# bioinformatics-ua/polus

Hardware: AMD Instinct MI355X
Metric: train samples/sec BioBERT-base NER seq256 (higher is better)
Workload: dtype bf16

## Files before the change

### polus_amd/csrc/attention.hip

```cpp
#include "common.h"

namespace {

constexpr int D = 64;
constexpr int BLK = 64;
constexpr float MASK_NEG = -10000.0f;
constexpr float LOG2E = 1.4426950408889634f, LN2 = 0.6931471805599453f;

template <typename T> struct TileCfg;
template <> struct TileCfg<bf16_t> { static constexpr int RS = 160, EPC = 8, LOG_CPR = 3, NLOAD = 2; };
template <> struct TileCfg<float> { static constexpr int RS = 288, EPC = 4, LOG_CPR = 4, NLOAD = 4; };

template <typename T, int NT = 256>
__device__ __forceinline__ void tile_load(unsigned char* tile, const T* __restrict__ base, long ld, int row0,
                                          int nrows, int col0, int tid) {
    constexpr int LOG = TileCfg<T>::LOG_CPR;
#pragma unroll
    for (int k = 0; k < TileCfg<T>::NLOAD; ++k) {
        int c = tid + NT * k;
        int r = c >> LOG, ch = c & ((1 << LOG) - 1);
        uint4 v = make_uint4(0, 0, 0, 0);
        if (row0 + r < nrows)
            v = *reinterpret_cast<const uint4*>(base + (long)(row0 + r) * ld + col0 + ch * TileCfg<T>::EPC);
        *reinterpret_cast<uint4*>(tile + r * TileCfg<T>::RS + ch * 16) = v;
    }
}

template <typename T>
__device__ __forceinline__ void frag_global(Frag<T>& f, const T* __restrict__ p, bool valid);
template <>
__device__ __forceinline__ void frag_global<bf16_t>(Frag<bf16_t>& f, const bf16_t* __restrict__ p, bool valid) {
    uint4 v = make_uint4(0, 0, 0, 0);
    if (valid) v = *reinterpret_cast<const uint4*>(p);
    f.v = __builtin_bit_cast(bf16x8, v);
}
template <>
__device__ __forceinline__ void frag_global<float>(Frag<float>& f, const float* __restrict__ p, bool valid) {
    float4 a = make_float4(0, 0, 0, 0), b = a;
    if (valid) { a = *reinterpret_cast<const float4*>(p); b = *reinterpret_cast<const float4*>(p + 4); }
    f.v[0] = a.x; f.v[1] = a.y; f.v[2] = a.z; f.v[3] = a.w;
    f.v[4] = b.x; f.v[5] = b.y; f.v[6] = b.z; f.v[7] = b.w;
}

template <typename T>
__device__ __forceinline__ void frag_row(Frag<T>& f, const unsigned char* tile, int row, int sub, int g) {
    frag_load_row(f, tile + row * TileCfg<T>::RS + (sub * 32 + 8 * g) * (int)sizeof(T));
}

__device__ __forceinline__ void frag_tr(Frag<bf16_t>& f, const unsigned char* tile, int kb, int d0, int i, int g) {
    const unsigned char* p = tile + (kb + 4 * g + (i >> 2)) * 160 + (d0 + 4 * (i & 3)) * 2;
    s16x4 lo = lds_tr16(p);
    s16x4 hi = lds_tr16(p + 16 * 160);
    typedef short s16x8 __attribute__((ext_vector_type(8)));
    s16x8 w = {lo[0], lo[1], lo[2], lo[3], hi[0], hi[1], hi[2], hi[3]};
    f.v = __builtin_bit_cast(bf16x8, w);
}
__device__ __forceinline__ void frag_tr(Frag<float>& f, const unsigned char* tile, int kb, int d0, int i, int g) {
#pragma unroll
    for (int j = 0; j < 8; ++j)
        f.v[j] = *reinterpret_cast<const float*>(tile + (kb + 16 * (j >> 2) + 4 * g + (j & 3)) * 288 + (d0 + i) * 4);
}

__device__ __forceinline__ void frag_from_acc(Frag<bf16_t>& f, const f32x4& t0, const f32x4& t1) {
    f.v[0] = (bf16_t)t0[0]; f.v[1] = (bf16_t)t0[1]; f.v[2] = (bf16_t)t0[2]; f.v[3] = (bf16_t)t0[3];
    f.v[4] = (bf16_t)t1[0]; f.v[5] = (bf16_t)t1[1]; f.v[6] = (bf16_t)t1[2]; f.v[7] = (bf16_t)t1[3];
}
__device__ __forceinline__ void frag_from_acc(Frag<float>& f, const f32x4& t0, const f32x4& t1) {
    f.v[0] = t0[0]; f.v[1] = t0[1]; f.v[2] = t0[2]; f.v[3] = t0[3];
    f.v[4] = t1[0]; f.v[5] = t1[1]; f.v[6] = t1[2]; f.v[7] = t1[3];
}

__device__ __forceinline__ float col_max(float v) { v = fmaxf(v, __shfl_xor(v, 16, 64)); return fmaxf(v, __shfl_xor(v, 32, 64)); }
__device__ __forceinline__ float col_sum(float v) { v += __shfl_xor(v, 16, 64); return v + __shfl_xor(v, 32, 64); }

template <typename T>
__device__ __forceinline__ void store_acc_T(T* __restrict__ out, long ld, int row, int col0, const f32x4 (&o)[4],
                                            float mul, int g, bool valid) {
    if (!valid) return;
#pragma unroll
    for (int dt = 0; dt < 4; ++dt) {
        float v[4] = {o[dt][0] * mul, o[dt][1] * mul, o[dt][2] * mul, o[dt][3] * mul};
        store4<T>(out + (long)row * ld + col0 + dt * 16 + 4 * g, v);
    }
}

struct AttnArgs {
    const void* qkv; const int32_t* mask; void* ctx; float* lse;
    const void* dctx; const float* delta; void* dqkv;
    int B, S, A, H;
    float scale;
    unsigned drop_thresh, drop_seed;
    float drop_inv;
    const PolusDyn* dyn;
    int debug;
};

__device__ __forceinline__ float key_bias(const int32_t* mask, int b, int S, int key) {
    if (key >= S) return -INFINITY;
    if (!mask) return 0.0f;
    return (1.0f - (float)mask[(long)b * S + key]) * MASK_NEG;
}

template <typename T, int NW>
__global__ __launch_bounds__(64 * NW) void attn_fwd_kernel(AttnArgs p) {
    if (p.drop_thresh) p.drop_seed = polus_eff_seed(p.drop_seed, p.dyn);
    constexpr int QB = 16 * NW, NT = 64 * NW;
    extern __shared__ __attribute__((aligned(16))) unsigned char smem[];
    unsigned char* Kc = smem;
    unsigned char* Vc = smem + QB * TileCfg<T>::RS;
    float* kbc = reinterpret_cast<float*>(smem + 2 * QB * TileCfg<T>::RS);
    const int tid = threadIdx.x, lane = tid & 63, wid = tid >> 6, i = lane & 15, g = lane >> 4;
    const int q0 = blockIdx.x * QB, h = blockIdx.y, b = blockIdx.z;
    const int S = p.S, H = p.H;
    const long ld = 3L * H;
    const T* qkv = static_cast<const T*>(p.qkv) + (long)b * S * ld;
    const int q = q0 + wid * 16 + i;
    const bool qvalid = q < S;

    Frag<T> qf[2];
#pragma unroll
    for (int sub = 0; sub < 2; ++sub)
        frag_global<T>(qf[sub], qkv + (long)q * ld + h * D + sub * 32 + 8 * g, qvalid);

    const float scale2 = p.scale * LOG2E;
    float m = -1e30f, l = 0.f;
    f32x4 o[4];
#pragma unroll
    for (int dt = 0; dt < 4; ++dt) o[dt] = (f32x4){0.f, 0.f, 0.f, 0.f};

    for (int kc0 = 0; kc0 < S; kc0 += QB) {
        __syncthreads();
        tile_load<T, NT>(Kc, qkv, ld, kc0, S, H + h * D, tid);
        tile_load<T, NT>(Vc, qkv, ld, kc0, S, 2 * H + h * D, tid);
        if (tid < QB) kbc[tid] = key_bias(p.mask, b, S, kc0 + tid) * LOG2E;
        __syncthreads();
      for (int kb0 = kc0; kb0 < kc0 + QB && kb0 < S; kb0 += BLK) {
        const unsigned char* Kt = Kc + (kb0 - kc0) * TileCfg<T>::RS;
        const unsigned char* Vt = Vc + (kb0 - kc0) * TileCfg<T>::RS;
        const float* kbias = kbc + (kb0 - kc0);

        f32x4 s[4];
#pragma unroll
        for (int kt = 0; kt < 4; ++kt) {
            s[kt] = (f32x4){0.f, 0.f, 0.f, 0.f};
#pragma unroll
            for (int sub = 0; sub < 2; ++sub) {
                Frag<T> a;
                frag_row<T>(a, Kt, kt * 16 + i, sub, g);
                mma16(s[kt], a, qf[sub]);
            }
        }
        float mx = -INFINITY;
#pragma unroll
        for (int kt = 0; kt < 4; ++kt)
#pragma unroll
            for (int r = 0; r < 4; ++r) {
                s[kt][r] = fmaf(s[kt][r], scale2, kbias[kt * 16 + 4 * g + r]);
                mx = fmaxf(mx, s[kt][r]);
            }
        mx = col_max(mx);
        const float m_new = fmaxf(m, mx);
        const float alpha = __builtin_amdgcn_exp2f(m - m_new);
        float rs = 0.f;
#pragma unroll
        for (int kt = 0; kt < 4; ++kt)
#pragma unroll
            for (int r = 0; r < 4; ++r) { s[kt][r] = __builtin_amdgcn_exp2f(s[kt][r] - m_new); rs += s[kt][r]; }
        rs = col_sum(rs);
        l = l * alpha + rs;
        m = m_new;
#pragma unroll
        for (int dt = 0; dt < 4; ++dt)
#pragma unroll
            for (int r = 0; r < 4; ++r) o[dt][r] *= alpha;
        if (p.drop_thresh) {
            const unsigned rowb = (((unsigned)b * p.A + h) * S + (unsigned)q) * S + kb0 + 4 * g;
#pragma unroll
            for (int kt = 0; kt < 4; ++kt) {
                float t4[4] = {s[kt][0], s[kt][1], s[kt][2], s[kt][3]};
                polus_dropout_run<4>(t4, p.drop_seed, rowb + kt * 16, p.drop_thresh, p.drop_inv, (S & 3) == 0);
                s[kt] = (f32x4){t4[0], t4[1], t4[2], t4[3]};
            }
        }
#pragma unroll
        for (int ks = 0; ks < 2; ++ks) {
            Frag<T> pb;
            frag_from_acc(pb, s[2 * ks], s[2 * ks + 1]);
#pragma unroll
            for (int dt = 0; dt < 4; ++dt) {
                Frag<T> va;
                frag_tr(va, Vt, ks * 32, dt * 16, i, g);
                mma16(o[dt], va, pb);
            }
        }
      }
    }
    T* ctx = static_cast<T*>(p.ctx) + (long)b * S * H;
    store_acc_T<T>(ctx, H, q, h * D, o, 1.0f / l, g, qvalid);
    if (qvalid && g == 0) p.lse[((long)b * p.A + h) * S + q] = m * LN2 + __logf(l);
}

typedef __attribute__((address_space(3))) void lds_void_t;
typedef const __attribute__((address_space(1))) void* gptr_t;
__device__ __forceinline__ void dma16(const void* g, unsigned char* lds) {
    __builtin_amdgcn_global_load_lds((gptr_t)g, (lds_void_t*)lds, 16, 0, 0);
}
__device__ __forceinline__ void dma4(const void* g, unsigned char* lds) {
    __builtin_amdgcn_global_load_lds((gptr_t)g, (lds_void_t*)lds, 4, 0, 0);
}
template <int N> __device__ __forceinline__ void wait_vm() { asm volatile("s_waitcnt vmcnt(%0)" :: "n"(N) : "memory"); }
__device__ __forceinline__ void wait_lgkm() { asm volatile("s_waitcnt lgkmcnt(0)" ::: "memory"); }
template <int PPW> __device__ __forceinline__ void wait_blocks_left(int left) {
    if (left >= 3) wait_vm<3 * PPW>(); else if (left == 2) wait_vm<2 * PPW>(); else if (left == 1) wait_vm<PPW>(); else wait_vm<0>();
}
__device__ __forceinline__ float xor16(float v) {
    return __builtin_bit_cast(float, __builtin_amdgcn_ds_swizzle(__builtin_bit_cast(int, v), 0x401F));
}
__device__ __forceinline__ float col_max2(float v) {
    v = fmaxf(v, xor16(v));
    return fmaxf(v, __shfl_xor(v, 32, 64));
}
__device__ __forceinline__ float col_sum2(float v) {
    v += xor16(v);
    return v + __shfl_xor(v, 32, 64);
}

constexpr int FWD_RING = 4, FWD_STAGE = 2 * BLK * 128;
constexpr int FWD_MAX_S = 1024;

template <int NW>
__global__ __launch_bounds__(64 * NW, NW == 8 ? 4 : 2) void attn_fwd_dma_kernel(AttnArgs p) {
    typedef bf16_t T;
    constexpr int QB = 16 * NW, NT = 64 * NW, PPW = 16 / NW;
    if (p.drop_thresh) p.drop_seed = polus_eff_seed(p.drop_seed, p.dyn);
    extern __shared__ __attribute__((aligned(16))) unsigned char smem[];
    unsigned char* ring = smem;
    float* kbc = reinterpret_cast<float*>(smem + FWD_RING * FWD_STAGE);
    const int tid = threadIdx.x, lane = tid & 63, i = lane & 15, g = lane >> 4;
    const int wid = __builtin_amdgcn_readfirstlane(tid >> 6);
    const int q0 = blockIdx.x * QB, h = blockIdx.y, b = blockIdx.z;
    const int S = p.S, H = p.H;
    const long ld = 3L * H;
    const T* qkv = static_cast<const T*>(p.qkv) + (long)b * S * ld;
    const int q = q0 + wid * 16 + i;
    const int r8 = lane >> 3, src_chunk = ((lane & 7) ^ r8) * 8;

    auto issue_block = [&](int j) {
        unsigned char* st = ring + (j & 3) * FWD_STAGE;
#pragma unroll
        for (int e = 0; e < PPW; ++e) {
            const int piece = wid + e * NW;
            const int row = min(j * BLK + (piece & 7) * 8 + r8, S - 1);
            dma16(qkv + (long)row * ld + (piece < 8 ? H : 2 * H) + h * D + src_chunk, st + piece * 1024);
        }
    };
    const int nblk = (S + BLK - 1) / BLK;
    if (p.mask)
        for (int k0 = wid * 64; k0 < S; k0 += 64 * NW)
            dma4(p.mask + (long)b * S + min(k0 + lane, S - 1), reinterpret_cast<unsigned char*>(kbc) + k0 * 4);
    {
        unsigned char* qs = ring + 3 * FWD_STAGE;
#pragma unroll
        for (int e = 0; e < 2; ++e) {
            const int piece = wid + e * NW;
            dma16(qkv + (long)min(q0 + piece * 8 + r8, S - 1) * ld + h * D + src_chunk, qs + piece * 1024);
        }
    }
#pragma unroll
    for (int j = 0; j < 3; ++j) if (j < nblk) issue_block(j);
    wait_blocks_left<PPW>(min(nblk, 3));
    __builtin_amdgcn_s_barrier();
    Frag<T> qf[2];
    {
        const int row = wid * 16 + i;
#pragma unroll
        for (int sub = 0; sub < 2; ++sub)
            qf[sub].v = *reinterpret_cast<const bf16x8*>(ring + 3 * FWD_STAGE + row * 128 + (((sub * 4 + g) ^ (row & 7)) * 16));
    }
    for (int t = tid; t < nblk * BLK; t += NT) {
        float bias = 0.0f;
        if (p.mask) bias = (1.0f - (float)reinterpret_cast<const int*>(kbc)[t]) * MASK_NEG;
        kbc[t] = t < S ? bias * LOG2E : -INFINITY;
    }
    wait_lgkm();
    __builtin_amdgcn_s_barrier();
    if (nblk > 3) issue_block(3);
    int issued = min(nblk, 4);

    const float scale2 = p.scale * LOG2E;
    float m = -1e30f, l = 0.f;
    f32x4 o[4];
#pragma unroll
    for (int dt = 0; dt < 4; ++dt) o[dt] = (f32x4){0.f, 0.f, 0.f, 0.f};
    const int kx = i & 7;
    const int k_off0 = i * 128 + ((g ^ kx) * 16), k_off1 = i * 128 + (((4 + g) ^ kx) * 16);
    const int vrow = 4 * g + (i >> 2), vx = vrow & 7;
    const int v_base = vrow * 128 + (i & 1) * 8, v_c = (i & 3) >> 1;

    for (int j0 = 0; j0 < nblk; j0 += 2) {
        const bool two = j0 + 1 < nblk;
        f32x4 s[2][4];
#pragma unroll
        for (int jj = 0; jj < 2; ++jj) {
            if (jj == 0 || two) {
                wait_blocks_left<PPW>(issued - 1 - (j0 + jj));
                __builtin_amdgcn_s_barrier();
                const unsigned char* Kt = ring + ((j0 + jj) & 3) * FWD_STAGE;
#pragma unroll
                for (int kt = 0; kt < 4; ++kt) {
                    s[jj][kt] = (f32x4){0.f, 0.f, 0.f, 0.f};
                    Frag<T> a0, a1;
                    a0.v = *reinterpret_cast<const bf16x8*>(Kt + kt * 2048 + k_off0);
                    a1.v = *reinterpret_cast<const bf16x8*>(Kt + kt * 2048 + k_off1);
                    mma16(s[jj][kt], a0, qf[0]);
                    mma16(s[jj][kt], a1, qf[1]);
                }
            } else {
#pragma unroll
                for (int kt = 0; kt < 4; ++kt) s[jj][kt] = (f32x4){-INFINITY, -INFINITY, -INFINITY, -INFINITY};
            }
        }
        float mx = -INFINITY;
#pragma unroll
        for (int jj = 0; jj < 2; ++jj)
            if (jj == 0 || two) {
#pragma unroll
                for (int kt = 0; kt < 4; ++kt) {
                    const f32x4 kb = *reinterpret_cast<const f32x4*>(kbc + (j0 + jj) * BLK + kt * 16 + 4 * g);
#pragma unroll
                    for (int r = 0; r < 4; ++r) s[jj][kt][r] = fmaf(s[jj][kt][r], scale2, kb[r]);
                    mx = fmaxf(mx, fmaxf(fmaxf(s[jj][kt][0], s[jj][kt][1]), fmaxf(s[jj][kt][2], s[jj][kt][3])));
                }
            }
        mx = col_max2(mx);
        const float m_new = fmaxf(m, mx);
        const float alpha = __builtin_amdgcn_exp2f(m - m_new);
        m = m_new;
        float rs = 0.f;
        Frag<T> pf[2][2];
#pragma unroll
        for (int jj = 0; jj < 2; ++jj) {
#pragma unroll
            for (int kt = 0; kt < 4; ++kt)
#pragma unroll
                for (int r = 0; r < 4; ++r) { s[jj][kt][r] = __builtin_amdgcn_exp2f(s[jj][kt][r] - m_new); rs += s[jj][kt][r]; }
            if (p.drop_thresh) {
                const unsigned rowb = (((unsigned)b * p.A + h) * S + (unsigned)q) * S + (j0 + jj) * BLK + 4 * g;
#pragma unroll
                for (int kt = 0; kt < 4; ++kt) {
                    float t4[4] = {s[jj][kt][0], s[jj][kt][1], s[jj][kt][2], s[jj][kt][3]};
                    polus_dropout_run<4>(t4, p.drop_seed, rowb + kt * 16, p.drop_thresh, p.drop_inv, (S & 3) == 0);
                    s[jj][kt] = (f32x4){t4[0], t4[1], t4[2], t4[3]};
                }
            }
            frag_from_acc(pf[jj][0], s[jj][0], s[jj][1]);
            frag_from_acc(pf[jj][1], s[jj][2], s[jj][3]);
        }
        l = l * alpha + rs;
#pragma unroll
        for (int dt = 0; dt < 4; ++dt)
#pragma unroll
            for (int r = 0; r < 4; ++r) o[dt][r] *= alpha;
#pragma unroll
        for (int jj = 0; jj < 2; ++jj) {
            if (jj == 0 || two) {
                const unsigned char* Vt = ring + ((j0 + jj) & 3) * FWD_STAGE + BLK * 128 + v_base;
#pragma unroll
                for (int ks = 0; ks < 2; ++ks)
#pragma unroll
                    for (int dt = 0; dt < 4; ++dt) {
                        const unsigned char* vp = Vt + ks * 4096 + (((2 * dt + v_c) ^ vx) * 16);
                        const s16x4 lo = lds_tr16(vp), hi = lds_tr16(vp + 16 * 128);
                        typedef short s16x8 __attribute__((ext_vector_type(8)));
                        const s16x8 w = {lo[0], lo[1], lo[2], lo[3], hi[0], hi[1], hi[2], hi[3]};
                        Frag<T> va;
                        va.v = __builtin_bit_cast(bf16x8, w);
                        mma16(o[dt], va, pf[jj][ks]);
                    }
            }
        }
        if (j0 + 4 < nblk) {
            wait_lgkm();
            __builtin_amdgcn_s_barrier();
            issue_block(j0 + 4);
            ++issued;
            if (j0 + 5 < nblk) { issue_block(j0 + 5); ++issued; }
        }
    }
    l = col_sum2(l);
    const float inv_l = 1.0f / l;
    wait_lgkm();
    __builtin_amdgcn_s_barrier();
    unsigned char* ot = ring + wid * 2048;
#pragma unroll
    for (int dt = 0; dt < 4; ++dt) {
        float v[4] = {o[dt][0] * inv_l, o[dt][1] * inv_l, o[dt][2] * inv_l, o[dt][3] * inv_l};
        store4<T>(reinterpret_cast<T*>(ot + i * 128 + (((2 * dt + (g >> 1)) ^ (i & 7)) * 16) + (g & 1) * 8), v);
    }
    wait_lgkm();
    T* ctx = static_cast<T*>(p.ctx) + (long)b * S * H;
#pragma unroll
    for (int t = 0; t < 2; ++t) {
        const int row = 8 * t + r8, qq = q0 + wid * 16 + row;
        const uint4 v = *reinterpret_cast<const uint4*>(ot + row * 128 + (lane & 7) * 16);
        if (qq < S) *reinterpret_cast<uint4*>(ctx + (long)qq * H + h * D + (((lane & 7) ^ (row & 7)) * 8)) = v;
    }
    if (q < S && g == 0) p.lse[((long)b * p.A + h) * S + q] = m * LN2 + __logf(l);
}

template <typename T, int NW>
__global__ __launch_bounds__(64 * NW) void attn_bwd_dq_kernel(AttnArgs p) {
    if (p.drop_thresh) p.drop_seed = polus_eff_seed(p.drop_seed, p.dyn);
    constexpr int QB = 16 * NW, NT = 64 * NW;
    extern __shared__ __attribute__((aligned(16))) unsigned char smem[];
    unsigned char* Kc = smem;
    unsigned char* Vc = smem + QB * TileCfg<T>::RS;
    float* kbc = reinterpret_cast<float*>(smem + 2 * QB * TileCfg<T>::RS);
    const int tid = threadIdx.x, lane = tid & 63, wid = tid >> 6, i = lane & 15, g = lane >> 4;
    const int q0 = blockIdx.x * QB, h = blockIdx.y, b = blockIdx.z;
    const int S = p.S, H = p.H;
    const long ld = 3L * H;
    const T* qkv = static_cast<const T*>(p.qkv) + (long)b * S * ld;
    const T* dctx = static_cast<const T*>(p.dctx) + (long)b * S * H;
    const int q = q0 + wid * 16 + i;
    const bool qvalid = q < S;

    Frag<T> qf[2], dof[2];
#pragma unroll
    for (int sub = 0; sub < 2; ++sub) {
        frag_global<T>(qf[sub], qkv + (long)q * ld + h * D + sub * 32 + 8 * g, qvalid);
        frag_global<T>(dof[sub], dctx + (long)q * H + h * D + sub * 32 + 8 * g, qvalid);
    }
    const long stat = ((long)b * p.A + h) * S + q;
    const float lse2 = (qvalid ? p.lse[stat] : 0.f) * LOG2E;
    const float scale2 = p.scale * LOG2E;
    float dl = 0.f;
    {
        const T* ctx = static_cast<const T*>(p.ctx) + (long)b * S * H;
#pragma unroll
        for (int sub = 0; sub < 2; ++sub) {
            Frag<T> of;
            frag_global<T>(of, ctx + (long)q * H + h * D + sub * 32 + 8 * g, qvalid);
#pragma unroll
            for (int j = 0; j < 8; ++j) dl += (float)of.v[j] * (float)dof[sub].v[j];
        }
        dl = col_sum(dl);
        if (qvalid && g == 0) const_cast<float*>(p.delta)[stat] = dl;
    }

    f32x4 dq[4];
#pragma unroll
    for (int dt = 0; dt < 4; ++dt) dq[dt] = (f32x4){0.f, 0.f, 0.f, 0.f};

    for (int kc0 = 0; kc0 < S; kc0 += QB) {
        __syncthreads();
        tile_load<T, NT>(Kc, qkv, ld, kc0, S, H + h * D, tid);
        tile_load<T, NT>(Vc, qkv, ld, kc0, S, 2 * H + h * D, tid);
        if (tid < QB) kbc[tid] = key_bias(p.mask, b, S, kc0 + tid) * LOG2E;
        __syncthreads();
      for (int kb0 = kc0; kb0 < kc0 + QB && kb0 < S; kb0 += BLK) {
        const unsigned char* Kt = Kc + (kb0 - kc0) * TileCfg<T>::RS;
        const unsigned char* Vt = Vc + (kb0 - kc0) * TileCfg<T>::RS;
        const float* kbias = kbc + (kb0 - kc0);
        f32x4 s[4], dp[4];
#pragma unroll
        for (int kt = 0; kt < 4; ++kt) {
            s[kt] = (f32x4){0.f, 0.f, 0.f, 0.f};
            dp[kt] = (f32x4){0.f, 0.f, 0.f, 0.f};
#pragma unroll
            for (int sub = 0; sub < 2; ++sub) {
                Frag<T> a;
                frag_row<T>(a, Kt, kt * 16 + i, sub, g);
                mma16(s[kt], a, qf[sub]);
                frag_row<T>(a, Vt, kt * 16 + i, sub, g);
                mma16(dp[kt], a, dof[sub]);
            }
            if (p.drop_thresh) {
                float t4[4] = {dp[kt][0], dp[kt][1], dp[kt][2], dp[kt][3]};
                const unsigned idx0 = (((unsigned)b * p.A + h) * S + (unsigned)q) * S + kb0 + kt * 16 + 4 * g;
                polus_dropout_run<4>(t4, p.drop_seed, idx0, p.drop_thresh, p.drop_inv, (S & 3) == 0);
                dp[kt] = (f32x4){t4[0], t4[1], t4[2], t4[3]};
            }
#pragma unroll
            for (int r = 0; r < 4; ++r) {
                float pr = __builtin_amdgcn_exp2f(fmaf(s[kt][r], scale2, kbias[kt * 16 + 4 * g + r]) - lse2);
                float dpe = dp[kt][r];
                s[kt][r] = pr * (dpe - dl) * p.scale;
            }
        }
#pragma unroll
        for (int ks = 0; ks < 2; ++ks) {
            Frag<T> dsb;
            frag_from_acc(dsb, s[2 * ks], s[2 * ks + 1]);
#pragma unroll
            for (int dt = 0; dt < 4; ++dt) {
                Frag<T> ka;
                frag_tr(ka, Kt, ks * 32, dt * 16, i, g);
                mma16(dq[dt], ka, dsb);
            }
        }
      }
    }
    T* dqkv = static_cast<T*>(p.dqkv) + (long)b * S * ld;
    store_acc_T<T>(dqkv, ld, q, h * D, dq, 1.0f, g, qvalid);
}

template <typename T>
__global__ __launch_bounds__(256, sizeof(T) == 2 ? 3 : 1) void attn_bwd_dkv_kernel(AttnArgs p) {
    if (p.drop_thresh) p.drop_seed = polus_eff_seed(p.drop_seed, p.dyn);
    constexpr int QCH = sizeof(T) == 2 ? 2 * BLK : BLK;
    __shared__ __attribute__((aligned(16))) unsigned char smem[2 * QCH * TileCfg<T>::RS + 2 * QCH * 4];
    unsigned char* Qc = smem;
    unsigned char* Oc = smem + QCH * TileCfg<T>::RS;
    float* lsec = reinterpret_cast<float*>(smem + 2 * QCH * TileCfg<T>::RS);
    float* deltac = lsec + QCH;
    const int tid = threadIdx.x, lane = tid & 63, wid = tid >> 6, i = lane & 15, g = lane >> 4;
    const int k0 = blockIdx.x * BLK, h = blockIdx.y, b = blockIdx.z;
    const int S = p.S, H = p.H;
    const long ld = 3L * H;
    const T* qkv = static_cast<const T*>(p.qkv) + (long)b * S * ld;
    const T* dctx = static_cast<const T*>(p.dctx) + (long)b * S * H;
    const int key = k0 + wid * 16 + i;
    const bool kvalid = key < S;

    Frag<T> kf[2], vf[2];
#pragma unroll
    for (int sub = 0; sub < 2; ++sub) {
        frag_global<T>(kf[sub], qkv + (long)key * ld + H + h * D + sub * 32 + 8 * g, kvalid);
        frag_global<T>(vf[sub], qkv + (long)key * ld + 2 * H + h * D + sub * 32 + 8 * g, kvalid);
    }
    const float kb2 = key_bias(p.mask, b, S, key) * LOG2E, scale2 = p.scale * LOG2E;
    const long stat0 = ((long)b * p.A + h) * S;

    f32x4 dk[4], dv[4];
#pragma unroll
    for (int dt = 0; dt < 4; ++dt) { dk[dt] = (f32x4){0.f, 0.f, 0.f, 0.f}; dv[dt] = (f32x4){0.f, 0.f, 0.f, 0.f}; }

    for (int qc0 = 0; qc0 < S; qc0 += QCH) {
        __syncthreads();
#pragma unroll
        for (int part = 0; part < QCH / BLK; ++part) {
            tile_load<T>(Qc + part * BLK * TileCfg<T>::RS, qkv, ld, qc0 + part * BLK, S, h * D, tid);
            tile_load<T>(Oc + part * BLK * TileCfg<T>::RS, dctx, H, qc0 + part * BLK, S, h * D, tid);
        }
        if (tid < QCH) {
            int qq = qc0 + tid;
            lsec[tid] = qq < S ? p.lse[stat0 + qq] * LOG2E : INFINITY;
            deltac[tid] = qq < S ? p.delta[stat0 + qq] : 0.f;
        }
        __syncthreads();
      for (int qb0 = qc0; qb0 < qc0 + QCH && qb0 < S; qb0 += BLK) {
        const unsigned char* Qt = Qc + (qb0 - qc0) * TileCfg<T>::RS;
        const unsigned char* Ot = Oc + (qb0 - qc0) * TileCfg<T>::RS;
        const float* slse = lsec + (qb0 - qc0);
        const float* sdelta = deltac + (qb0 - qc0);
        f32x4 s[4], dp[4];
#pragma unroll
        for (int qt = 0; qt < 4; ++qt) {
            s[qt] = (f32x4){0.f, 0.f, 0.f, 0.f};
            dp[qt] = (f32x4){0.f, 0.f, 0.f, 0.f};
#pragma unroll
            for (int sub = 0; sub < 2; ++sub) {
                Frag<T> a;
                frag_row<T>(a, Qt, qt * 16 + i, sub, g);
                mma16(s[qt], a, kf[sub]);
                frag_row<T>(a, Ot, qt * 16 + i, sub, g);
                mma16(dp[qt], a, vf[sub]);
            }
#pragma unroll
            for (int r = 0; r < 4; ++r) {
                int ql = qt * 16 + 4 * g + r;
                float pr = __builtin_amdgcn_exp2f(fmaf(s[qt][r], scale2, kb2) - slse[ql]);
                float dpe = dp[qt][r], pd = pr;
                if (p.drop_thresh) {
                    const unsigned idx = (((unsigned)b * p.A + h) * S + (unsigned)(qb0 + ql)) * S + (unsigned)key;
                    const bool keep = polus_keep(p.drop_seed, idx, p.drop_thresh);
                    dpe = keep ? dpe * p.drop_inv : 0.f;
                    pd = keep ? pr * p.drop_inv : 0.f;
                }
                dp[qt][r] = pr * (dpe - sdelta[ql]) * p.scale;
                s[qt][r] = pd;
            }
        }
#pragma unroll
        for (int ks = 0; ks < 2; ++ks) {
            Frag<T> pb, dsb;
            frag_from_acc(pb, s[2 * ks], s[2 * ks + 1]);
            frag_from_acc(dsb, dp[2 * ks], dp[2 * ks + 1]);
#pragma unroll
            for (int dt = 0; dt < 4; ++dt) {
                Frag<T> a;
                frag_tr(a, Ot, ks * 32, dt * 16, i, g);
                mma16(dv[dt], a, pb);
                frag_tr(a, Qt, ks * 32, dt * 16, i, g);
                mma16(dk[dt], a, dsb);
            }
        }
      }
    }
    T* dqkv = static_cast<T*>(p.dqkv) + (long)b * S * ld;
    store_acc_T<T>(dqkv, ld, key, H + h * D, dk, 1.0f, g, kvalid);
    store_acc_T<T>(dqkv, ld, key, 2 * H + h * D, dv, 1.0f, g, kvalid);
}

constexpr int KBLK = 32, RSS = 64;

__device__ __forceinline__ void frag_tr_rs(Frag<bf16_t>& f, const unsigned char* tile, int rs, int kb, int c0, int i, int g) {
    const unsigned char* p = tile + (kb + 4 * g + (i >> 2)) * rs + (c0 + 4 * (i & 3)) * 2;
    s16x4 lo = lds_tr16(p);
    s16x4 hi = lds_tr16(p + 16 * rs);
    typedef short s16x8 __attribute__((ext_vector_type(8)));
    s16x8 w = {lo[0], lo[1], lo[2], lo[3], hi[0], hi[1], hi[2], hi[3]};
    f.v = __builtin_bit_cast(bf16x8, w);
}

template <int NW>
__global__ __launch_bounds__(64 * NW) void attn_bwd_fused_kernel(AttnArgs p) {
    typedef bf16_t T;
    constexpr int S = 16 * NW, NT = 64 * NW, RS = TileCfg<T>::RS, NKB = S / KBLK, TPW = 16 / NW;
    if (p.drop_thresh) p.drop_seed = polus_eff_seed(p.drop_seed, p.dyn);
    extern __shared__ __attribute__((aligned(16))) unsigned char smem[];
    unsigned char* Qc = smem;
    unsigned char* Oc = Qc + S * RS;
    unsigned char* Kc = Oc + S * RS;
    unsigned char* Vc = Kc + 2 * KBLK * RS;
    unsigned char* Ps = Vc + 2 * KBLK * RS;
    unsigned char* Ds = Ps + S * RSS;
    float* kbc = reinterpret_cast<float*>(Ds + S * RSS);
    const int tid = threadIdx.x, lane = tid & 63, wid = tid >> 6, i = lane & 15, g = lane >> 4;
    const int h = blockIdx.x, b = blockIdx.y;
    const int H = p.H;
    const long ld = 3L * H;
    const T* qkv = static_cast<const T*>(p.qkv) + (long)b * S * ld;
    const T* dctx = static_cast<const T*>(p.dctx) + (long)b * S * H;
    T* dqkv = static_cast<T*>(p.dqkv) + (long)b * S * ld;
    const int q = wid * 16 + i;

    auto load_kv = [&](int kb, int buf) {
        for (int c = tid; c < 2 * KBLK * 8; c += NT) {
            const int which = c >> 8, cc = c & 255, r = cc >> 3, ch = cc & 7;
            const uint4 v = *reinterpret_cast<const uint4*>(qkv + (long)(kb * KBLK + r) * ld + (1 + which) * H + h * D + ch * 8);
            *reinterpret_cast<uint4*>((which ? Vc : Kc) + (buf * KBLK + r) * RS + ch * 16) = v;
        }
    };
    tile_load<T, NT>(Qc, qkv, ld, 0, S, h * D, tid);
    tile_load<T, NT>(Oc, dctx, H, 0, S, h * D, tid);
    load_kv(0, 0);
    if (tid < S) kbc[tid] = key_bias(p.mask, b, S, tid) * LOG2E;

    Frag<T> qf[2], dof[2];
#pragma unroll
    for (int sub = 0; sub < 2; ++sub) {
        frag_global<T>(qf[sub], qkv + (long)q * ld + h * D + sub * 32 + 8 * g, true);
        frag_global<T>(dof[sub], dctx + (long)q * H + h * D + sub * 32 + 8 * g, true);
    }
    const long stat = ((long)b * p.A + h) * S + q;
    const float lse2 = p.lse[stat] * LOG2E;
    const float scale2 = p.scale * LOG2E;
    float dl = 0.f;
    {
        const T* ctx = static_cast<const T*>(p.ctx) + (long)b * S * H;
#pragma unroll
        for (int sub = 0; sub < 2; ++sub) {
            Frag<T> of;
            frag_global<T>(of, ctx + (long)q * H + h * D + sub * 32 + 8 * g, true);
#pragma unroll
            for (int j = 0; j < 8; ++j) dl += (float)of.v[j] * (float)dof[sub].v[j];
        }
        dl = col_sum(dl);
    }
    f32x4 dq[4];
#pragma unroll
    for (int dt = 0; dt < 4; ++dt) dq[dt] = (f32x4){0.f, 0.f, 0.f, 0.f};
    __syncthreads();

    for (int kb = 0; kb < NKB; ++kb) {
        const int cur = kb & 1;
        const unsigned char* Kt = Kc + cur * KBLK * RS;
        const unsigned char* Vt = Vc + cur * KBLK * RS;
        if (kb + 1 < NKB) load_kv(kb + 1, cur ^ 1);
        f32x4 s[2], dp[2];
#pragma unroll
        for (int kt = 0; kt < 2; ++kt) {
            s[kt] = (f32x4){0.f, 0.f, 0.f, 0.f};
            dp[kt] = (f32x4){0.f, 0.f, 0.f, 0.f};
#pragma unroll
            for (int sub = 0; sub < 2; ++sub) {
                Frag<T> a;
                frag_row<T>(a, Kt, kt * 16 + i, sub, g);
                mma16(s[kt], a, qf[sub]);
                frag_row<T>(a, Vt, kt * 16 + i, sub, g);
                mma16(dp[kt], a, dof[sub]);
            }
        }
        const unsigned rowb = (((unsigned)b * p.A + h) * S + (unsigned)q) * S + kb * KBLK + 4 * g;
#pragma unroll
        for (int kt = 0; kt < 2; ++kt) {
            float pd[4], dsv[4];
            bool keep[4] = {true, true, true, true};
            if (p.drop_thresh) {
                polus_keep4(p.drop_seed, rowb + kt * 16, p.drop_thresh, keep);
            }
#pragma unroll
            for (int r = 0; r < 4; ++r) {
                const float pr = __builtin_amdgcn_exp2f(fmaf(s[kt][r], scale2, kbc[kb * KBLK + kt * 16 + 4 * g + r]) - lse2);
                const float pk = keep[r] ? pr * p.drop_inv : 0.f;
                const float dpe = keep[r] ? dp[kt][r] * p.drop_inv : 0.f;
                pd[r] = pk;
                dsv[r] = pr * (dpe - dl) * p.scale;
                s[kt][r] = dsv[r];
            }
            const int st_off = kt * (S * 32) + q * 32 + ((g ^ ((q >> 2) & 3)) * 8);
            store4<T>(reinterpret_cast<T*>(Ps + st_off), pd);
            store4<T>(reinterpret_cast<T*>(Ds + st_off), dsv);
        }
        {
            Frag<T> dsb;
            frag_from_acc(dsb, s[0], s[1]);
#pragma unroll
            for (int dt = 0; dt < 4; ++dt) {
                Frag<T> ka;
                frag_tr(ka, Kt, 0, dt * 16, i, g);
                mma16(dq[dt], ka, dsb);
            }
        }
        __syncthreads();
#pragma unroll
        for (int e = 0; e < TPW; ++e) {
            const int t = wid * TPW + e;
            const int type = t >> 3, dt = (t >> 1) & 3, ktile = t & 1;
            const unsigned char* At = type ? Oc : Qc;
            const unsigned char* Bt = type ? Ps : Ds;
            f32x4 acc = (f32x4){0.f, 0.f, 0.f, 0.f};
#pragma unroll
            for (int qs = 0; qs < S / 32; ++qs) {
                Frag<T> a, bb;
                frag_tr(a, At, qs * 32, dt * 16, i, g);
                {
                    const unsigned char* bp = Bt + ktile * (S * 32) + (qs * 32 + 4 * g + (i >> 2)) * 32 + (((i & 3) ^ g) * 8);
                    const s16x4 lo = lds_tr16(bp), hi = lds_tr16(bp + 16 * 32);
                    typedef short s16x8 __attribute__((ext_vector_type(8)));
                    const s16x8 w = {lo[0], lo[1], lo[2], lo[3], hi[0], hi[1], hi[2], hi[3]};
                    bb.v = __builtin_bit_cast(bf16x8, w);
                }
                mma16(acc, a, bb);
            }
            float v[4] = {acc[0], acc[1], acc[2], acc[3]};
            store4<T>(dqkv + (long)(kb * KBLK + ktile * 16 + i) * ld + (type ? 2 * H : H) + h * D + dt * 16 + 4 * g, v);
        }
        __syncthreads();
    }
    store_acc_T<T>(dqkv, ld, q, h * D, dq, 1.0f, g, true);
}

typedef __attribute__((address_space(3))) unsigned char lds_u8;
typedef int v2i_t __attribute__((ext_vector_type(2)));
__device__ __forceinline__ unsigned lds_off(const unsigned char* p) { return (unsigned)(unsigned long)(const lds_u8*)p; }
template <int ROW16>
__device__ __forceinline__ void tr_pair_asm(Frag<bf16_t>& f, unsigned addr) {
    v2i_t lo, hi;
    asm volatile("ds_read_b64_tr_b16 %0, %2\n\tds_read_b64_tr_b16 %1, %2 offset:%3" : "=&v"(lo), "=&v"(hi) : "v"(addr), "n"(ROW16));
    typedef int v4i_t __attribute__((ext_vector_type(4)));
    const v4i_t w = {lo[0], lo[1], hi[0], hi[1]};
    f.v = __builtin_bit_cast(bf16x8, w);
}
__device__ __forceinline__ void ds_read128_asm(Frag<bf16_t>& f, unsigned addr) {
    typedef int v4i_t __attribute__((ext_vector_type(4)));
    v4i_t w;
    asm volatile("ds_read_b128 %0, %1" : "=&v"(w) : "v"(addr));
    f.v = __builtin_bit_cast(bf16x8, w);
}
__device__ __forceinline__ uint2 ds_read64_asm(unsigned addr) {
    v2i_t w;
    asm volatile("ds_read_b64 %0, %1" : "=&v"(w) : "v"(addr));
    return make_uint2((unsigned)w[0], (unsigned)w[1]);
}
__device__ __forceinline__ void lds_fence() {
    asm volatile("s_waitcnt lgkmcnt(0)" ::: "memory");
    __builtin_amdgcn_sched_barrier(0);
}
template <int R> __device__ __forceinline__ unsigned quad_bcast(unsigned v) {
    return (unsigned)__builtin_amdgcn_mov_dpp((int)v, R | (R << 2) | (R << 4) | (R << 6), 0xF, 0xF, true);
}


constexpr int Q64_KB = 64;
template <int NW> struct Q64Cfg {
    static constexpr int S = 16 * NW;
    static constexpr int OFF_O = S * 128, OFF_K = 2 * S * 128, OFF_V = OFF_K + Q64_KB * 128, OFF_P = OFF_V + Q64_KB * 128,
                         OFF_D = OFF_P + 4 * S * 32, OFF_B = OFF_D + 4 * S * 32, SMEM = OFF_B + S * 4;
};

template <int NW>
__global__ __launch_bounds__(64 * NW, 4) void attn_bwd_q64_kernel(AttnArgs p) {
    typedef bf16_t T;
    typedef Q64Cfg<NW> C;
    constexpr int S = C::S, NT = 64 * NW, NKB = S / Q64_KB;
    constexpr int KVP = 16 / NW;
    constexpr int COMBOS = NW >= 8 ? 1 : 8 / NW;
    constexpr int KTW = NW == 16 ? 2 : 4;
    if (p.drop_thresh) p.drop_seed = polus_eff_seed(p.drop_seed, p.dyn);
    extern __shared__ __attribute__((aligned(16))) unsigned char smem[];
    unsigned char* Qi = smem;
    unsigned char* Oi = smem + C::OFF_O;
    unsigned char* Kb = smem + C::OFF_K;
    unsigned char* Vb = smem + C::OFF_V;
    unsigned char* Ps = smem + C::OFF_P;
    unsigned char* Ds = smem + C::OFF_D;
    float* kbc = reinterpret_cast<float*>(smem + C::OFF_B);
    const int tid = threadIdx.x, lane = tid & 63, i = lane & 15, g = lane >> 4;
    const int wid = __builtin_amdgcn_readfirstlane(tid >> 6);
    const int h = blockIdx.x, b = blockIdx.y;
    const int H = p.H;
    const long ld = 3L * H;
    const T* qkv = static_cast<const T*>(p.qkv) + (long)b * S * ld;
    const T* dctx = static_cast<const T*>(p.dctx) + (long)b * S * H;
    T* dqkv = static_cast<T*>(p.dqkv) + (long)b * S * ld;
    const int q = wid * 16 + i;
    const int r8 = lane >> 3, src_chunk = ((lane & 7) ^ r8) * 8;

    auto issue_kv = [&](int kb) {
#pragma unroll
        for (int e = 0; e < KVP; ++e) {
            const int piece = wid + e * NW;
            const long row = (long)(kb * Q64_KB + (piece & 7) * 8 + r8) * ld + h * D + src_chunk;
            dma16(qkv + row + (piece < 8 ? H : 2 * H), (piece < 8 ? Kb : Vb) + (piece & 7) * 1024);
        }
    };
#pragma unroll
    for (int e = 0; e < 2; ++e) {
        const int piece = wid + e * NW;
        dma16(qkv + (long)(piece * 8 + r8) * ld + h * D + src_chunk, Qi + piece * 1024);
        dma16(dctx + (long)(piece * 8 + r8) * H + h * D + src_chunk, Oi + piece * 1024);
    }
    issue_kv(0);
    if (tid < S) kbc[tid] = key_bias(p.mask, b, S, tid) * LOG2E;
    const long stat = ((long)b * p.A + h) * S + q;
    const float lse2 = p.lse[stat] * LOG2E;
    const float scale2 = p.scale * LOG2E;
    Frag<T> of[2];
    {
        const T* ctx = static_cast<const T*>(p.ctx) + (long)b * S * H;
#pragma unroll
        for (int sub = 0; sub < 2; ++sub) frag_global<T>(of[sub], ctx + (long)q * H + h * D + sub * 32 + 8 * g, true);
    }
    wait_vm<0>();
    wait_lgkm();
    __builtin_amdgcn_s_barrier();
    const int qoff0 = q * 128 + ((g ^ (q & 7)) * 16), qoff1 = q * 128 + (((4 + g) ^ (q & 7)) * 16);
    float dl = 0.f;
    {
        Frag<T> dof[2];
        ds_read128_asm(dof[0], lds_off(Oi + qoff0));
        ds_read128_asm(dof[1], lds_off(Oi + qoff1));
        lds_fence();
#pragma unroll
        for (int sub = 0; sub < 2; ++sub)
#pragma unroll
            for (int j = 0; j < 8; ++j) dl += (float)of[sub].v[j] * (float)dof[sub].v[j];
        dl = col_sum(dl);
    }
    f32x4 dq[4];
#pragma unroll
    for (int dt = 0; dt < 4; ++dt) dq[dt] = (f32x4){0.f, 0.f, 0.f, 0.f};

    const int rr0 = i * 128 + ((g ^ (i & 7)) * 16), rr1 = i * 128 + (((4 + g) ^ (i & 7)) * 16);
    const int trow = 4 * g + (i >> 2), tx = trow & 7, thalf = (i & 1) * 8, tc = (i & 3) >> 1;
    const int st_w = q * 32 + ((g ^ ((q >> 2) & 3)) * 8);
    const int st_r = trow * 32 + (((i & 3) ^ g) * 8);

    for (int kb = 0; kb < NKB; ++kb) {
        f32x4 s[4];
        Frag<T> qf[2], dof[2];
        ds_read128_asm(qf[0], lds_off(Qi + qoff0));
        ds_read128_asm(qf[1], lds_off(Qi + qoff1));
        ds_read128_asm(dof[0], lds_off(Oi + qoff0));
        ds_read128_asm(dof[1], lds_off(Oi + qoff1));
        const unsigned rowb = (((unsigned)b * p.A + h) * S + (unsigned)q) * S + kb * Q64_KB + 4 * g;
#pragma unroll
        for (int kt = 0; kt < 4; ++kt) {
            Frag<T> ka[2], va[2];
            ds_read128_asm(ka[0], lds_off(Kb + kt * 2048 + rr0));
            ds_read128_asm(ka[1], lds_off(Kb + kt * 2048 + rr1));
            ds_read128_asm(va[0], lds_off(Vb + kt * 2048 + rr0));
            ds_read128_asm(va[1], lds_off(Vb + kt * 2048 + rr1));
            lds_fence();
            f32x4 dp = (f32x4){0.f, 0.f, 0.f, 0.f};
            s[kt] = (f32x4){0.f, 0.f, 0.f, 0.f};
            mma16(s[kt], ka[0], qf[0]);
            mma16(s[kt], ka[1], qf[1]);
            mma16(dp, va[0], dof[0]);
            mma16(dp, va[1], dof[1]);
            float pd[4], dsv[4];
            bool keep[4] = {true, true, true, true};
            if (p.drop_thresh) polus_keep4(p.drop_seed, rowb + kt * 16, p.drop_thresh, keep);
            const f32x4 kbv = *reinterpret_cast<const f32x4*>(kbc + kb * Q64_KB + kt * 16 + 4 * g);
#pragma unroll
            for (int r = 0; r < 4; ++r) {
                const float pr = __builtin_amdgcn_exp2f(fmaf(s[kt][r], scale2, kbv[r]) - lse2);
                const float pk = keep[r] ? pr * p.drop_inv : 0.f;
                const float dpe = keep[r] ? dp[r] * p.drop_inv : 0.f;
                pd[r] = pk;
                dsv[r] = pr * (dpe - dl) * p.scale;
                s[kt][r] = dsv[r];
            }
            store4<T>(reinterpret_cast<T*>(Ps + kt * (S * 32) + st_w), pd);
            store4<T>(reinterpret_cast<T*>(Ds + kt * (S * 32) + st_w), dsv);
        }
        {
            Frag<T> kT[2][4];
#pragma unroll
            for (int ks = 0; ks < 2; ++ks)
#pragma unroll
                for (int dt = 0; dt < 4; ++dt)
                    tr_pair_asm<16 * 128>(kT[ks][dt], lds_off(Kb + (ks * 32 + trow) * 128 + (((2 * dt + tc) ^ tx) * 16) + thalf));
            lds_fence();
#pragma unroll
            for (int ks = 0; ks < 2; ++ks) {
                Frag<T> dsb;
                frag_from_acc(dsb, s[2 * ks], s[2 * ks + 1]);
#pragma unroll
                for (int dt = 0; dt < 4; ++dt) mma16(dq[dt], kT[ks][dt], dsb);
            }
        }
        wait_lgkm();
        __builtin_amdgcn_s_barrier();
        if (kb + 1 < NKB) issue_kv(kb + 1);
#pragma unroll
        for (int c = 0; c < COMBOS; ++c) {
            const int combo = NW == 16 ? (wid >> 1) : wid * COMBOS + c;
            const int type = combo >> 2, dt = combo & 3, kt0 = NW == 16 ? (wid & 1) * 2 : 0;
            const unsigned char* At = type ? Oi : Qi;
            const unsigned char* Bt = type ? Ps : Ds;
            constexpr int QH = (S / 32) < 4 ? (S / 32) : 4;
            f32x4 acc[KTW];
#pragma unroll
            for (int k2 = 0; k2 < KTW; ++k2) acc[k2] = (f32x4){0.f, 0.f, 0.f, 0.f};
#pragma unroll
            for (int q0 = 0; q0 < S / 32; q0 += QH) {
                Frag<T> af[QH];
#pragma unroll
                for (int qs = 0; qs < QH; ++qs)
                    tr_pair_asm<16 * 128>(af[qs], lds_off(At + ((q0 + qs) * 32 + trow) * 128 + (((2 * dt + tc) ^ tx) * 16) + thalf));
#pragma unroll
                for (int k2 = 0; k2 < KTW; ++k2) {
                    Frag<T> bf[QH];
#pragma unroll
                    for (int qs = 0; qs < QH; ++qs)
                        tr_pair_asm<16 * 32>(bf[qs], lds_off(Bt + (kt0 + k2) * (S * 32) + (q0 + qs) * 32 * 32 + st_r));
                    lds_fence();
#pragma unroll
                    for (int qs = 0; qs < QH; ++qs) mma16(acc[k2], af[qs], bf[qs]);
                }
            }
#pragma unroll
            for (int k2 = 0; k2 < KTW; ++k2) {
                float v[4] = {acc[k2][0], acc[k2][1], acc[k2][2], acc[k2][3]};
                store4<T>(dqkv + (long)(kb * Q64_KB + (kt0 + k2) * 16 + i) * ld + (type ? 2 * H : H) + h * D + dt * 16 + 4 * g, v);
            }
        }
        if (kb + 1 < NKB) wait_vm<COMBOS * KTW>();
        wait_lgkm();
        __builtin_amdgcn_s_barrier();
    }
    store_acc_T<T>(dqkv, ld, q, h * D, dq, 1.0f, g, true);
}

constexpr int KR_KEYS = 256, KR_QS = 32, KR_RING = 4;
constexpr int KR_KV = KR_KEYS * 128;
constexpr int KR_SLICE = KR_QS * 128;
constexpr int KR_DS = 2 * KR_KEYS * 32;
constexpr int KR_OFF_RING = 2 * KR_KV, KR_OFF_DS = KR_OFF_RING + KR_RING * 2 * KR_SLICE, KR_OFF_DQ = KR_OFF_DS + 2 * KR_DS,
              KR_OFF_STAT = KR_OFF_DQ + 2 * KR_SLICE;

__global__ __launch_bounds__(512, 2) void attn_bwd_kres_kernel(AttnArgs p, float* __restrict__ dq_slabs) {
    typedef bf16_t T;
    constexpr int NT = 512;
    if (p.drop_thresh) p.drop_seed = polus_eff_seed(p.drop_seed, p.dyn);
    extern __shared__ __attribute__((aligned(16))) unsigned char smem[];
    unsigned char* Kimg = smem;
    unsigned char* Vimg = smem + KR_KV;
    unsigned char* ring = smem + KR_OFF_RING;
    unsigned char* dsb = smem + KR_OFF_DS;
    unsigned char* dqb = smem + KR_OFF_DQ;
    float* lsec = reinterpret_cast<float*>(smem + KR_OFF_STAT);
    const int S = p.S, H = p.H;
    float* deltac = lsec + S;
    const int tid = threadIdx.x, lane = tid & 63, i = lane & 15, g = lane >> 4;
    const int wid = __builtin_amdgcn_readfirstlane(tid >> 6);
    const int kb = blockIdx.x, h = blockIdx.y, b = blockIdx.z;
    const int key0 = kb * KR_KEYS;
    const long ld = 3L * H;
    const T* qkv = static_cast<const T*>(p.qkv) + (long)b * S * ld;
    const T* dctx = static_cast<const T*>(p.dctx) + (long)b * S * H;
    T* dqkv = static_cast<T*>(p.dqkv) + (long)b * S * ld;
    const int r8 = lane >> 3, src_chunk = ((lane & 7) ^ r8) * 8;
    const int nsl = S / KR_QS;

#pragma unroll
    for (int e = 0; e < 4; ++e) {
        const int piece = wid + 8 * e;
        const long row = (long)(key0 + piece * 8 + r8) * ld + h * D + src_chunk;
        dma16(qkv + row + H, Kimg + piece * 1024);
        dma16(qkv + row + 2 * H, Vimg + piece * 1024);
    }
    auto issue_slice = [&](int t) {
        const int q = t * KR_QS + (wid & 3) * 8 + r8;
        unsigned char* dst = ring + (t & 3) * 2 * KR_SLICE + wid * 1024;
        if (wid < 4) dma16(qkv + (long)q * ld + h * D + src_chunk, dst);
        else dma16(dctx + (long)q * H + h * D + src_chunk, dst);
    };
#pragma unroll
    for (int t = 0; t < 3; ++t) if (t < nsl) issue_slice(t);
    {
        const T* ctx = static_cast<const T*>(p.ctx) + (long)b * S * H;
        const long stat0 = ((long)b * p.A + h) * S;
        for (int q8 = wid * 8; q8 < S; q8 += 256) {
            bf16x8 o[4], d[4];
#pragma unroll
            for (int u = 0; u < 4; ++u) {
                const int q = q8 + 64 * u + r8;
                if (!(p.debug & 8)) {
                    o[u] = *reinterpret_cast<const bf16x8*>(ctx + (long)q * H + h * D + (lane & 7) * 8);
                    d[u] = *reinterpret_cast<const bf16x8*>(dctx + (long)q * H + h * D + (lane & 7) * 8);
                } else { o[u] = (bf16x8)(bf16_t)0.f; d[u] = o[u]; }
            }
            float l4[4];
            if ((lane & 7) == 0) {
#pragma unroll
                for (int u = 0; u < 4; ++u) l4[u] = p.lse[stat0 + q8 + 64 * u + r8];
            }
#pragma unroll
            for (int u = 0; u < 4; ++u) {
                float dl = 0.f;
#pragma unroll
                for (int j = 0; j < 8; ++j) dl += (float)o[u][j] * (float)d[u][j];
                dl += __builtin_bit_cast(float, __builtin_amdgcn_ds_swizzle(__builtin_bit_cast(int, dl), 0x041F));
                dl += __builtin_bit_cast(float, __builtin_amdgcn_ds_swizzle(__builtin_bit_cast(int, dl), 0x081F));
                dl += __builtin_bit_cast(float, __builtin_amdgcn_ds_swizzle(__builtin_bit_cast(int, dl), 0x101F));
                if ((lane & 7) == 0) { deltac[q8 + 64 * u + r8] = dl; lsec[q8 + 64 * u + r8] = l4[u] * LOG2E; }
            }
        }
    }
    float kb2[2];
#pragma unroll
    for (int kt = 0; kt < 2; ++kt) kb2[kt] = key_bias(p.mask, b, S, key0 + wid * 32 + kt * 16 + i) * LOG2E;
    wait_vm<0>();
    wait_lgkm();
    __builtin_amdgcn_s_barrier();

    const int my_dt = wid & 3, my_qt = wid >> 2;
    Frag<T> kf[2][2], vf[2][2], ktr[8];
#pragma unroll
    for (int kt = 0; kt < 2; ++kt)
#pragma unroll
        for (int sub = 0; sub < 2; ++sub) {
            const int row = wid * 32 + kt * 16 + i, off = row * 128 + (((sub * 4 + g) ^ (row & 7)) * 16);
            ds_read128_asm(kf[kt][sub], lds_off(Kimg + off));
            ds_read128_asm(vf[kt][sub], lds_off(Vimg + off));
        }
    const int trow = 4 * g + (i >> 2), tx = trow & 7, thalf = (i & 1) * 8, tc = (i & 3) >> 1;
#pragma unroll
    for (int ks = 0; ks < 8; ++ks)
        tr_pair_asm<16 * 128>(ktr[ks], lds_off(Kimg + (ks * 32 + trow) * 128 + (((2 * my_dt + tc) ^ tx) * 16) + thalf));
    lds_fence();
#pragma unroll
    for (int ks = 0; ks < 8; ++ks)
#pragma unroll
        for (int j = 0; j < 8; ++j) ktr[ks].v[j] = (bf16_t)((float)ktr[ks].v[j] * p.scale);

    f32x4 dk[4][2], dv[4][2];
#pragma unroll
    for (int dt = 0; dt < 4; ++dt)
#pragma unroll
        for (int kt = 0; kt < 2; ++kt) { dk[dt][kt] = (f32x4){0.f, 0.f, 0.f, 0.f}; dv[dt][kt] = (f32x4){0.f, 0.f, 0.f, 0.f}; }
    const float scale2 = p.scale * LOG2E;
    const int rr_off0 = i * 128 + ((g ^ (i & 7)) * 16), rr_off1 = i * 128 + (((4 + g) ^ (i & 7)) * 16);
    int ds_w[2];
#pragma unroll
    for (int kt = 0; kt < 2; ++kt) { const int row = wid * 32 + kt * 16 + i; ds_w[kt] = row * 32 + ((g ^ ((row >> 2) & 3)) * 8); }
    const int ds_r = my_qt * (KR_KEYS * 32) + trow * 32 + (((i & 3) ^ (g & 3)) * 8);
    const unsigned hash_row = ((unsigned)b * p.A + h) * S;
    const int my_r = i & 3;

    f32x4 dq_prev = (f32x4){0.f, 0.f, 0.f, 0.f};
    for (int t = 0; t < nsl; ++t) {
        const unsigned char* sl = ring + (t & 3) * 2 * KR_SLICE;
        const int q0 = t * KR_QS;
        Frag<T> qr[2][2], dor[2][2];
#pragma unroll
        for (int qt = 0; qt < 2; ++qt) {
            ds_read128_asm(qr[qt][0], lds_off(sl + qt * 2048 + rr_off0));
            ds_read128_asm(qr[qt][1], lds_off(sl + qt * 2048 + rr_off1));
            ds_read128_asm(dor[qt][0], lds_off(sl + KR_SLICE + qt * 2048 + rr_off0));
            ds_read128_asm(dor[qt][1], lds_off(sl + KR_SLICE + qt * 2048 + rr_off1));
        }
        lds_fence();
        f32x4 s[2][2], dp[2][2];
#pragma unroll
        for (int qt = 0; qt < 2; ++qt)
#pragma unroll
            for (int kt = 0; kt < 2; ++kt) {
                s[qt][kt] = (f32x4){0.f, 0.f, 0.f, 0.f};
                dp[qt][kt] = (f32x4){0.f, 0.f, 0.f, 0.f};
                mma16(s[qt][kt], qr[qt][0], kf[kt][0]);
                mma16(s[qt][kt], qr[qt][1], kf[kt][1]);
                mma16(dp[qt][kt], dor[qt][0], vf[kt][0]);
                mma16(dp[qt][kt], dor[qt][1], vf[kt][1]);
            }
        Frag<T> qT[4], doT[4];
#pragma unroll
        for (int dt = 0; dt < 4; ++dt) {
            const int off = trow * 128 + (((2 * dt + tc) ^ tx) * 16) + thalf;
            tr_pair_asm<16 * 128>(qT[dt], lds_off(sl + off));
            tr_pair_asm<16 * 128>(doT[dt], lds_off(sl + KR_SLICE + off));
        }
        Frag<T> pf[2], dsf[2];
        if (!(p.debug & 2))
#pragma unroll
        for (int qt = 0; qt < 2; ++qt) {
            const f32x4 l2 = *reinterpret_cast<const f32x4*>(lsec + q0 + qt * 16 + 4 * g);
            const f32x4 de = *reinterpret_cast<const f32x4*>(deltac + q0 + qt * 16 + 4 * g);
#pragma unroll
            for (int kt = 0; kt < 2; ++kt) {
                unsigned h1 = 0, h2 = 0;
                if (p.drop_thresh) {
                    const unsigned key = key0 + wid * 32 + kt * 16 + i;
                    const unsigned idx = (hash_row + (unsigned)(q0 + qt * 16 + 4 * g + my_r)) * (unsigned)S + (key & ~3u);
                    h1 = polus_hash32(p.drop_seed, idx >> 2);
                    h2 = polus_hash32_second(h1);
                }
                float pd[4], dsv[4];
#pragma unroll
                for (int r = 0; r < 4; ++r) {
                    const float pr = __builtin_amdgcn_exp2f(fmaf(s[qt][kt][r], scale2, kb2[kt]) - l2[r]);
                    float pk = pr, dpe = dp[qt][kt][r];
                    if (p.drop_thresh) {
                        const unsigned a1 = r == 0 ? quad_bcast<0>(h1) : r == 1 ? quad_bcast<1>(h1) : r == 2 ? quad_bcast<2>(h1) : quad_bcast<3>(h1);
                        const unsigned a2 = r == 0 ? quad_bcast<0>(h2) : r == 1 ? quad_bcast<1>(h2) : r == 2 ? quad_bcast<2>(h2) : quad_bcast<3>(h2);
                        const unsigned hh = (i & 2) ? a2 : a1;
                        const bool keep = ((i & 1) ? (hh >> 16) : (hh & 0xFFFFu)) >= p.drop_thresh;
                        pk = keep ? pr * p.drop_inv : 0.f;
                        dpe = keep ? dpe * p.drop_inv : 0.f;
                    }
                    pd[r] = pk;
                    dsv[r] = pr * (dpe - de[r]);
                }
                s[qt][kt] = (f32x4){pd[0], pd[1], pd[2], pd[3]};
                dp[qt][kt] = (f32x4){dsv[0], dsv[1], dsv[2], dsv[3]};
                store4<T>(reinterpret_cast<T*>(dsb + (t & 1) * KR_DS + qt * (KR_KEYS * 32) + ds_w[kt]), dsv);
            }
        }
#pragma unroll
        for (int kt = 0; kt < 2; ++kt) {
            frag_from_acc(pf[kt], s[0][kt], s[1][kt]);
            frag_from_acc(dsf[kt], dp[0][kt], dp[1][kt]);
        }
        lds_fence();
        if (!(p.debug & 4))
#pragma unroll
        for (int dt = 0; dt < 4; ++dt)
#pragma unroll
            for (int kt = 0; kt < 2; ++kt) {
                mma16(dv[dt][kt], doT[dt], pf[kt]);
                mma16(dk[dt][kt], qT[dt], dsf[kt]);
            }
        {
            const int younger = (t >= 2 ? 1 : 0) + (t + 2 < nsl ? 1 : 0);
            if (younger >= 2) wait_vm<2>(); else if (younger == 1) wait_vm<1>(); else wait_vm<0>();
        }
        wait_lgkm();
        __builtin_amdgcn_s_barrier();
        if (t >= 1 && dq_slabs) {
            float* dst = dq_slabs + ((long)kb * p.B * S + (long)b * S + q0 - KR_QS + my_qt * 16 + i) * H + h * D + my_dt * 16 + 4 * g;
            *reinterpret_cast<float4*>(dst) = make_float4(dq_prev[0], dq_prev[1], dq_prev[2], dq_prev[3]);
        }
        if (t >= 1 && !dq_slabs && !(p.debug & 16)) {
            const unsigned char* src = dqb + ((t - 1) & 1) * KR_SLICE;
            const int row = tid >> 4, c8 = tid & 15;
            const uint2 v = ds_read64_asm(lds_off(src + row * 128 + (((c8 >> 1) ^ (row & 7)) * 16) + (c8 & 1) * 8));
            lds_fence();
            *reinterpret_cast<uint2*>(dqkv + (long)(q0 - KR_QS + row) * ld + h * D + c8 * 4) = v;
        }
        if (t + 3 < nsl) issue_slice(t + 3);
        f32x4 dq = (f32x4){0.f, 0.f, 0.f, 0.f};
        if (!(p.debug & 1)) {
            Frag<T> dst[8];
            const unsigned base = lds_off(dsb + (t & 1) * KR_DS + ds_r);
#pragma unroll
            for (int ks = 0; ks < 8; ++ks) tr_pair_asm<16 * 32>(dst[ks], base + ks * 32 * 32);
            lds_fence();
#pragma unroll
            for (int ks = 0; ks < 8; ++ks) mma16(dq, ktr[ks], dst[ks]);
        }
        dq_prev = dq;
        if (!dq_slabs) {
            float v[4] = {dq[0], dq[1], dq[2], dq[3]};
            const int row = my_qt * 16 + i;
            store4<T>(reinterpret_cast<T*>(dqb + (t & 1) * KR_SLICE + row * 128 + (((2 * my_dt + (g >> 1)) ^ (row & 7)) * 16) + (g & 1) * 8), v);
        }
    }
    wait_lgkm();
    __builtin_amdgcn_s_barrier();
    if (dq_slabs) {
        float* dst = dq_slabs + ((long)kb * p.B * S + (long)b * S + (nsl - 1) * KR_QS + my_qt * 16 + i) * H + h * D + my_dt * 16 + 4 * g;
        *reinterpret_cast<float4*>(dst) = make_float4(dq_prev[0], dq_prev[1], dq_prev[2], dq_prev[3]);
    }
    if (!dq_slabs) {
        const unsigned char* src = dqb + ((nsl - 1) & 1) * KR_SLICE;
        const int row = tid >> 4, c8 = tid & 15;
        const uint2 v = *reinterpret_cast<const uint2*>(src + row * 128 + (((c8 >> 1) ^ (row & 7)) * 16) + (c8 & 1) * 8);
        *reinterpret_cast<uint2*>(dqkv + (long)((nsl - 1) * KR_QS + row) * ld + h * D + c8 * 4) = v;
    }
#pragma unroll
    for (int kt = 0; kt < 2; ++kt) {
        const long key = key0 + wid * 32 + kt * 16 + i;
#pragma unroll
        for (int dt = 0; dt < 4; ++dt) {
            float a[4] = {dk[dt][kt][0] * p.scale, dk[dt][kt][1] * p.scale, dk[dt][kt][2] * p.scale, dk[dt][kt][3] * p.scale};
            float c[4] = {dv[dt][kt][0], dv[dt][kt][1], dv[dt][kt][2], dv[dt][kt][3]};
            store4<T>(dqkv + key * ld + H + h * D + dt * 16 + 4 * g, a);
            store4<T>(dqkv + key * ld + 2 * H + h * D + dt * 16 + 4 * g, c);
        }
    }
}

__global__ __launch_bounds__(256) void attn_bwd_dq_finish_kernel(const float* __restrict__ slabs, bf16_t* __restrict__ dqkv,
                                                                  long rows, int H, int nkb) {
    const long n4 = rows * (H / 4);
    for (long e = (long)blockIdx.x * blockDim.x + threadIdx.x; e < n4; e += (long)gridDim.x * blockDim.x) {
        const long row = e / (H / 4);
        const int c = (int)(e - row * (H / 4)) * 4;
        float4 a = *reinterpret_cast<const float4*>(slabs + row * H + c);
        for (int k = 1; k < nkb; ++k) {
            const float4 v = *reinterpret_cast<const float4*>(slabs + ((long)k * rows + row) * H + c);
            a.x += v.x; a.y += v.y; a.z += v.z; a.w += v.w;
        }
        float v[4] = {a.x, a.y, a.z, a.w};
        store4<bf16_t>(dqkv + row * 3L * H + c, v);
    }
}

int check_common(const char* who, int dtype, int B, int S, int A, int hd) {
    POLUS_REQUIRE(dtype == POLUS_F32 || dtype == POLUS_BF16, "%s: bad dtype %d", who, dtype);
    POLUS_REQUIRE(hd == D, "%s: head_dim must be 64 (got %d)", who, hd);
    POLUS_REQUIRE(B > 0 && S > 0 && A > 0, "%s: bad shape B=%d S=%d A=%d", who, B, S, A);
    POLUS_REQUIRE(B <= 65535 && A <= 65535, "%s: B and n_heads must be <= 65535", who);
    return POLUS_OK;
}

}

namespace {
template <int WHICH, typename T, int NW>
int launch_wide_nw(const AttnArgs& a, hipStream_t st) {
    auto kern = WHICH == 0 ? attn_fwd_kernel<T, NW> : attn_bwd_dq_kernel<T, NW>;
    constexpr int QB = 16 * NW;
    const size_t lds = 2 * (size_t)QB * TileCfg<T>::RS + QB * 4;
    static bool attr_done = false;
    if (!attr_done && lds > 48 * 1024) {
        POLUS_HIP(hipFuncSetAttribute(reinterpret_cast<const void*>(kern), hipFuncAttributeMaxDynamicSharedMemorySize, (int)lds));
        attr_done = true;
    }
    dim3 grid((a.S + QB - 1) / QB, a.A, a.B);
    hipLaunchKernelGGL(kern, grid, dim3(64 * NW), lds, st, a);
    return POLUS_OK;
}
template <int NW>
int launch_fwd_dma(const AttnArgs& a, hipStream_t st) {
    auto kern = attn_fwd_dma_kernel<NW>;
    const size_t lds = FWD_RING * FWD_STAGE + (size_t)((a.S + 64 * NW - 1) / (64 * NW)) * 64 * NW * 4;
    static bool attr_done = false;
    if (!attr_done) {
        POLUS_HIP(hipFuncSetAttribute(reinterpret_cast<const void*>(kern), hipFuncAttributeMaxDynamicSharedMemorySize,
                                      FWD_RING * FWD_STAGE + (FWD_MAX_S + 64 * NW) * 4));
        attr_done = true;
    }
    hipLaunchKernelGGL(kern, dim3((a.S + 16 * NW - 1) / (16 * NW), a.A, a.B), dim3(64 * NW), lds, st, a);
    return POLUS_OK;
}
template <int NW>
int launch_q64(const AttnArgs& a, int n_heads, int B, hipStream_t st) {
    auto kern = attn_bwd_q64_kernel<NW>;
    static bool attr_done = false;
    if (!attr_done) {
        POLUS_HIP(hipFuncSetAttribute(reinterpret_cast<const void*>(kern), hipFuncAttributeMaxDynamicSharedMemorySize, Q64Cfg<NW>::SMEM));
        attr_done = true;
    }
    hipLaunchKernelGGL(kern, dim3(n_heads, B), dim3(64 * NW), Q64Cfg<NW>::SMEM, st, a);
    return POLUS_OK;
}
template <int NW>
int launch_fused(const AttnArgs& a, int n_heads, int B, size_t lds, hipStream_t st) {
    auto kern = attn_bwd_fused_kernel<NW>;
    static bool attr_done = false;
    if (!attr_done) {
        POLUS_HIP(hipFuncSetAttribute(reinterpret_cast<const void*>(kern), hipFuncAttributeMaxDynamicSharedMemorySize, (int)lds));
        attr_done = true;
    }
    hipLaunchKernelGGL(kern, dim3(n_heads, B), dim3(64 * NW), lds, st, a);
    return POLUS_OK;
}
template <int WHICH>
int launch_wide(int dtype, const AttnArgs& a, hipStream_t st) {
    if (dtype != POLUS_BF16) return launch_wide_nw<WHICH, float, 4>(a, st);
    if (a.S >= 96) return launch_wide_nw<WHICH, bf16_t, 8>(a, st);
    return launch_wide_nw<WHICH, bf16_t, 4>(a, st);
}
}

extern "C" int polus_attention_fwd(int dtype, const void* qkv, const int32_t* mask, void* ctx, float* lse,
                                   int B, int S, int n_heads, int head_dim, float drop_p, uint32_t seed, void* stream) {
    int rc = check_common("polus_attention_fwd", dtype, B, S, n_heads, head_dim);
    if (rc) return rc;
    POLUS_REQUIRE(qkv && ctx && lse, "polus_attention_fwd: null pointer");
    POLUS_REQUIRE(polus_aligned16(qkv) && polus_aligned16(ctx), "polus_attention_fwd: pointers must be 16-byte aligned");
    AttnArgs a = {};
    POLUS_REQUIRE(drop_p >= 0.f && drop_p < 1.f && (long)B * n_heads * S * S < (1LL << 32), "polus_attention_fwd: bad dropout arguments");
    a.qkv = qkv; a.mask = mask; a.ctx = ctx; a.lse = lse;
    a.B = B; a.S = S; a.A = n_heads; a.H = n_heads * D; a.scale = 0.125f;
    a.drop_thresh = drop_p > 0.f ? polus_drop_thresh(drop_p) : 0u; a.drop_seed = seed; a.drop_inv = 1.0f / (1.0f - drop_p); a.dyn = polus_dyn();
    hipStream_t st = static_cast<hipStream_t>(stream);
    int rc2;
    if (dtype == POLUS_BF16 && S <= FWD_MAX_S)
        rc2 = S >= 96 ? launch_fwd_dma<8>(a, st) : launch_fwd_dma<4>(a, st);
    else
        rc2 = launch_wide<0>(dtype, a, st);
    if (rc2 != POLUS_OK) return rc2;
    POLUS_CHECK_LAUNCH("polus_attention_fwd");
    return POLUS_OK;
}

extern "C" size_t polus_attention_bwd_workspace_bytes(int B, int S, int n_heads) {
    size_t n = (size_t)B * S * n_heads * sizeof(float);
    if (S > KR_KEYS && S % KR_KEYS == 0 && S <= 2048) n += (size_t)(S / KR_KEYS) * B * S * n_heads * D * sizeof(float);
    return n;
}

extern "C" int polus_attention_bwd(int dtype, const void* qkv, const int32_t* mask, const void* ctx,
                                   const void* dctx, const float* lse, void* dqkv,
                                   int B, int S, int n_heads, int head_dim, float drop_p, uint32_t seed,
                                   void* workspace, size_t workspace_bytes, void* stream) {
    int rc = check_common("polus_attention_bwd", dtype, B, S, n_heads, head_dim);
    if (rc) return rc;
    POLUS_REQUIRE(qkv && ctx && dctx && lse && dqkv, "polus_attention_bwd: null pointer");
    POLUS_REQUIRE(polus_aligned16(qkv) && polus_aligned16(ctx) && polus_aligned16(dctx) && polus_aligned16(dqkv),
                  "polus_attention_bwd: pointers must be 16-byte aligned");
    size_t need = polus_attention_bwd_workspace_bytes(B, S, n_heads);
    if (!workspace || workspace_bytes < need) { polus_set_error("polus_attention_bwd: workspace %zu < %zu", workspace_bytes, need); return POLUS_ERR_WORKSPACE; }
    AttnArgs a = {};
    a.qkv = qkv; a.mask = mask; a.ctx = const_cast<void*>(ctx); a.lse = const_cast<float*>(lse); a.dctx = dctx; a.dqkv = dqkv;
    a.delta = static_cast<const float*>(workspace);
    a.B = B; a.S = S; a.A = n_heads; a.H = n_heads * D; a.scale = 0.125f;
    POLUS_REQUIRE(drop_p >= 0.f && drop_p < 1.f, "polus_attention_bwd: bad drop_p");
    a.drop_thresh = drop_p > 0.f ? polus_drop_thresh(drop_p) : 0u; a.drop_seed = seed; a.drop_inv = 1.0f / (1.0f - drop_p); a.dyn = polus_dyn();
    a.debug = polus_cfg().attn_debug;
    hipStream_t st = static_cast<hipStream_t>(stream);
    dim3 grid((S + BLK - 1) / BLK, n_heads, B);
    const int kres = polus_cfg().attn_bwd_kres;
    if (dtype == POLUS_BF16 && polus_cfg().attn_fused && kres && S % KR_KEYS == 0 && S <= 2048 && (S > KR_KEYS || kres >= 2)) {
        const int nkb = S / KR_KEYS;
        float* slabs = nkb > 1 ? static_cast<float*>(workspace) + (size_t)B * S * n_heads : nullptr;
        const size_t lds = KR_OFF_STAT + 2 * (size_t)S * sizeof(float);
        static bool attr_done = false;
        if (!attr_done) {
            POLUS_HIP(hipFuncSetAttribute(reinterpret_cast<const void*>(attn_bwd_kres_kernel), hipFuncAttributeMaxDynamicSharedMemorySize, 160 * 1024));
            attr_done = true;
        }
        hipLaunchKernelGGL(attn_bwd_kres_kernel, dim3(nkb, n_heads, B), dim3(512), lds, st, a, slabs);
        POLUS_CHECK_LAUNCH("polus_attention_bwd(key-resident)");
        if (nkb > 1) {
            hipLaunchKernelGGL(attn_bwd_dq_finish_kernel, dim3(1024), dim3(256), 0, st, slabs, static_cast<bf16_t*>(dqkv), (long)B * S, a.H, nkb);
            POLUS_CHECK_LAUNCH("polus_attention_bwd(dQ slabs)");
        }
        return POLUS_OK;
    }
    const int fused = polus_cfg().attn_fused;
    if (dtype == POLUS_BF16 && fused && S == 256) {
        int rc2 = launch_q64<16>(a, n_heads, B, st);
        if (rc2 != POLUS_OK) return rc2;
        POLUS_CHECK_LAUNCH("polus_attention_bwd(one pass, 64-key blocks)");
        return POLUS_OK;
    }
    if (dtype == POLUS_BF16 && fused && (S == 64 || S == 128)) {
        const size_t lds = 2 * (size_t)S * TileCfg<bf16_t>::RS + 4 * (size_t)KBLK * TileCfg<bf16_t>::RS + 2 * (size_t)S * RSS + (size_t)S * 4;
        int rc2 = S == 128 ? launch_fused<8>(a, n_heads, B, lds, st) : launch_fused<4>(a, n_heads, B, lds, st);
        if (rc2 != POLUS_OK) return rc2;
        POLUS_CHECK_LAUNCH("polus_attention_bwd(fused)");
        return POLUS_OK;
    }
    if (dtype == POLUS_BF16) {
        { int rc2 = launch_wide<1>(dtype, a, st); if (rc2 != POLUS_OK) return rc2; }
        POLUS_CHECK_LAUNCH("polus_attention_bwd(dq)");
        hipLaunchKernelGGL(attn_bwd_dkv_kernel<bf16_t>, grid, dim3(256), 0, st, a);
    } else {
        { int rc2 = launch_wide<1>(dtype, a, st); if (rc2 != POLUS_OK) return rc2; }
        POLUS_CHECK_LAUNCH("polus_attention_bwd(dq)");
        hipLaunchKernelGGL(attn_bwd_dkv_kernel<float>, grid, dim3(256), 0, st, a);
    }
    POLUS_CHECK_LAUNCH("polus_attention_bwd(dkv)");
    return POLUS_OK;
}
```

### polus_amd/csrc/common.h

```cpp
#pragma once
#include <hip/hip_runtime.h>
#include <stdint.h>
#include <stdio.h>
#include <string.h>
#include <math.h>

#include "../../include/polus_hip.h"

typedef __bf16 bf16_t;
typedef __bf16 bf16x8 __attribute__((ext_vector_type(8)));
typedef __bf16 bf16x4 __attribute__((ext_vector_type(4)));
typedef short s16x4 __attribute__((ext_vector_type(4)));
typedef float f32x4 __attribute__((ext_vector_type(4)));

void polus_set_error(const char* fmt, ...);
#define POLUS_FAIL(...) do { polus_set_error(__VA_ARGS__); return POLUS_ERR_INVALID; } while (0)
#define POLUS_REQUIRE(cond, ...) do { if (!(cond)) { polus_set_error(__VA_ARGS__); return POLUS_ERR_INVALID; } } while (0)
#define POLUS_CHECK_LAUNCH(name) do { hipError_t e__ = hipGetLastError(); \
    if (e__ != hipSuccess) { polus_set_error("%s: launch failed: %s", name, hipGetErrorString(e__)); return POLUS_ERR_HIP; } } while (0)
#define POLUS_HIP(call) do { hipError_t e__ = (call); \
    if (e__ != hipSuccess) { polus_set_error("%s failed: %s", #call, hipGetErrorString(e__)); return POLUS_ERR_HIP; } } while (0)

static inline size_t polus_dtype_size(int dt) { return dt == POLUS_BF16 ? 2 : 4; }
static inline bool polus_aligned16(const void* p) { return (((uintptr_t)p) & 15) == 0; }

struct PolusCfg {
    int gemm_pp;
    int gemm_v1;
    int dw_ungrouped;
    int dw_fused_reduce;
    int ln_bwd_blocks;
    int ln_fin_single;
    int gemm_ring128;
    int gemm_auto_split;
    int ln_halfwave;
    int gemm_order;
    int gemm_persist;
    int reserve_cus;
    int attn_bwd_kres;
    int attn_debug;
    int dw_streamk;
    int dw_sk_cus;
    int dw_sk_delta;
    int attn_fused;
};
const PolusCfg& polus_cfg();
int polus_num_cus();
int polus_reserved_cus();

struct PolusDyn { uint32_t salt; float lr, lr_t; uint32_t pad; };
const PolusDyn* polus_dyn();
__device__ __forceinline__ uint32_t polus_eff_seed(uint32_t seed, const PolusDyn* dyn) {
    if (!dyn) return seed;
    uint32_t x = seed + dyn->salt;
    x ^= x >> 15;
    return x * 0x2C1B3C6Du;
}

template <typename T> __device__ __forceinline__ float to_f(T x);
template <> __device__ __forceinline__ float to_f<float>(float x) { return x; }
template <> __device__ __forceinline__ float to_f<bf16_t>(bf16_t x) { return (float)x; }
template <typename T> __device__ __forceinline__ T from_f(float x);
template <> __device__ __forceinline__ float from_f<float>(float x) { return x; }
template <> __device__ __forceinline__ bf16_t from_f<bf16_t>(float x) { return (bf16_t)x; }

template <typename T> __device__ __forceinline__ void load4(const T* p, float (&v)[4]);
template <> __device__ __forceinline__ void load4<float>(const float* p, float (&v)[4]) {
    float4 t = *reinterpret_cast<const float4*>(p); v[0] = t.x; v[1] = t.y; v[2] = t.z; v[3] = t.w;
}
template <> __device__ __forceinline__ void load4<bf16_t>(const bf16_t* p, float (&v)[4]) {
    bf16x4 t = *reinterpret_cast<const bf16x4*>(p);
    v[0] = (float)t[0]; v[1] = (float)t[1]; v[2] = (float)t[2]; v[3] = (float)t[3];
}
template <typename T> __device__ __forceinline__ void store4(T* p, const float (&v)[4]);
template <> __device__ __forceinline__ void store4<float>(float* p, const float (&v)[4]) {
    *reinterpret_cast<float4*>(p) = make_float4(v[0], v[1], v[2], v[3]);
}
template <> __device__ __forceinline__ void store4<bf16_t>(bf16_t* p, const float (&v)[4]) {
    bf16x4 t; t[0] = (bf16_t)v[0]; t[1] = (bf16_t)v[1]; t[2] = (bf16_t)v[2]; t[3] = (bf16_t)v[3];
    *reinterpret_cast<bf16x4*>(p) = t;
}

__device__ __forceinline__ float erf_fast(float x) {
    const float ax = fabsf(x);
    const float t = __frcp_rn(1.0f + 0.3275911f * ax);
    float poly = 1.061405429f;
    poly = poly * t - 1.453152027f;
    poly = poly * t + 1.421413741f;
    poly = poly * t - 0.284496736f;
    poly = poly * t + 0.254829592f;
    const float r = 1.0f - poly * t * __expf(-ax * ax);
    return copysignf(r, x);
}
__device__ __forceinline__ float gelu_f(float x) { return 0.5f * x * (1.0f + erf_fast(x * 0.70710678118654752f)); }
__device__ __forceinline__ float gelu_grad_f(float x) {
    float cdf = 0.5f * (1.0f + erf_fast(x * 0.70710678118654752f));
    float pdf = 0.3989422804014327f * __expf(-0.5f * x * x);
    return cdf + x * pdf;
}
__device__ __forceinline__ float swish_f(float x) { return x / (1.0f + __expf(-x)); }
__device__ __forceinline__ float swish_grad_f(float x) {
    float s = 1.0f / (1.0f + __expf(-x));
    return s * (1.0f + x * (1.0f - s));
}
typedef float f32x2_t __attribute__((ext_vector_type(2)));
__device__ __forceinline__ f32x2_t gelu_poly2(f32x2_t x, const float (&c)[11]) {
    f32x2_t xc = {__builtin_amdgcn_fmed3f(x[0], -4.5f, 4.5f), __builtin_amdgcn_fmed3f(x[1], -4.5f, 4.5f)};
    f32x2_t s = xc * xc;
    f32x2_t u = __builtin_elementwise_fma(s, (f32x2_t){2.0f / 20.25f, 2.0f / 20.25f}, (f32x2_t){-1.0f, -1.0f});
    f32x2_t r = {c[10], c[10]};
#pragma unroll
    for (int k = 9; k >= 0; --k) r = __builtin_elementwise_fma(r, u, (f32x2_t){c[k], c[k]});
    return __builtin_elementwise_fma(xc, r, (f32x2_t){0.5f, 0.5f});
}
__device__ __forceinline__ f32x2_t gelu_cdf2(f32x2_t x) {
    const float q[11] = {1.569049305e-01f, -7.719386095e-02f, 5.470119065e-02f, -4.010921159e-02f, 2.828393083e-02f,
                         -1.902094059e-02f, 1.143922652e-02f, -5.251548121e-03f, 2.716277400e-03f, -2.340015935e-03f,
                         9.806926012e-04f};
    return gelu_poly2(x, q);
}
__device__ __forceinline__ f32x2_t gelu_grad2(f32x2_t x) {
    const float w[11] = {1.594289755e-01f, -9.003904569e-02f, 8.714168751e-02f, -9.350841452e-02f, 9.645831298e-02f,
                         -9.557466143e-02f, 7.437658385e-02f, -3.356380937e-02f, 2.252388123e-02f, -3.068672777e-02f,
                         1.457471506e-02f};
    return gelu_poly2(x, w);
}
template <int N, bool FAST = false> __device__ __forceinline__ void apply_act_n(int act, float (&v)[N]) {
    if (act == POLUS_ACT_GELU) {
        if (FAST && (N % 2) == 0) {
#pragma unroll
            for (int r = 0; r < N; r += 2) {
                f32x2_t x = {v[r], v[r + 1]};
                f32x2_t y = x * gelu_cdf2(x);
                v[r] = y[0]; v[r + 1] = y[1];
            }
            return;
        }
#pragma unroll
        for (int r = 0; r < N; ++r) v[r] = gelu_f(v[r]);
    } else if (act == POLUS_ACT_SWISH) {
#pragma unroll
        for (int r = 0; r < N; ++r) v[r] = swish_f(v[r]);
    } else if (act == POLUS_ACT_RELU) {
#pragma unroll
        for (int r = 0; r < N; ++r) v[r] = fmaxf(v[r], 0.0f);
    } else if (act == POLUS_ACT_TANH) {
#pragma unroll
        for (int r = 0; r < N; ++r) v[r] = tanhf(v[r]);
    }
}
template <int N, bool FAST = false> __device__ __forceinline__ void apply_act_grad_n(int act, float (&v)[N], const float (&u)[N]) {
    if (act == POLUS_ACT_GELU) {
        if (FAST && (N % 2) == 0) {
#pragma unroll
            for (int r = 0; r < N; r += 2) {
                f32x2_t d = (f32x2_t){v[r], v[r + 1]} * gelu_grad2((f32x2_t){u[r], u[r + 1]});
                v[r] = d[0]; v[r + 1] = d[1];
            }
            return;
        }
#pragma unroll
        for (int r = 0; r < N; ++r) v[r] *= gelu_grad_f(u[r]);
    } else if (act == POLUS_ACT_SWISH) {
#pragma unroll
        for (int r = 0; r < N; ++r) v[r] *= swish_grad_f(u[r]);
    } else if (act == POLUS_ACT_RELU) {
#pragma unroll
        for (int r = 0; r < N; ++r) v[r] = u[r] > 0.0f ? v[r] : 0.0f;
    } else if (act == POLUS_ACT_TANH) {
#pragma unroll
        for (int r = 0; r < N; ++r) { float t = tanhf(u[r]); v[r] *= 1.0f - t * t; }
    }
}

__device__ __forceinline__ uint32_t polus_hash32(uint32_t seed, uint32_t idx) {
    uint32_t x = idx * 0x9E3779B1u + seed;
    x ^= x >> 16; x *= 0x85EBCA6Bu;
    x ^= x >> 13; x *= 0xC2B2AE35u;
    x ^= x >> 16;
    return x;
}
__device__ __forceinline__ uint32_t polus_hash32_second(uint32_t h1) {
    uint32_t y = h1 * 0x27D4EB2Fu;
    return y ^ (y >> 15);
}
__device__ __forceinline__ bool polus_keep(uint32_t seed, uint32_t idx, uint32_t thresh) {
    const uint32_t h1 = polus_hash32(seed, idx >> 2);
    const uint32_t h = (idx & 2u) ? polus_hash32_second(h1) : h1;
    return ((idx & 1u) ? (h >> 16) : (h & 0xFFFFu)) >= thresh;
}
__device__ __forceinline__ void polus_keep4(uint32_t seed, uint32_t idx4, uint32_t thresh, bool (&k)[4]) {
    const uint32_t h1 = polus_hash32(seed, idx4 >> 2), h2 = polus_hash32_second(h1);
    k[0] = (h1 & 0xFFFFu) >= thresh;
    k[1] = (h1 >> 16) >= thresh;
    k[2] = (h2 & 0xFFFFu) >= thresh;
    k[3] = (h2 >> 16) >= thresh;
}
template <int N>
__device__ __forceinline__ void polus_dropout_run(float (&v)[N], uint32_t seed, uint32_t base, uint32_t thresh, float inv, bool quad) {
    static_assert(N % 4 == 0, "runs of whole quads");
    if (quad) {
#pragma unroll
        for (int r = 0; r < N; r += 4) {
            bool k[4];
            polus_keep4(seed, base + r, thresh, k);
#pragma unroll
            for (int e = 0; e < 4; ++e) v[r + e] = k[e] ? v[r + e] * inv : 0.f;
        }
    } else {
#pragma unroll
        for (int r = 0; r < N; ++r) v[r] = polus_keep(seed, base + r, thresh) ? v[r] * inv : 0.f;
    }
}
static inline uint32_t polus_drop_thresh(float p) {
    double t = (double)p * 65536.0 + 0.5;
    return t <= 0.0 ? 0u : (t >= 65535.0 ? 65535u : (uint32_t)t);
}

__device__ __forceinline__ float wave_sum(float v) {
#pragma unroll
    for (int o = 32; o > 0; o >>= 1) v += __shfl_xor(v, o, 64);
    return v;
}
__device__ __forceinline__ float wave_max(float v) {
#pragma unroll
    for (int o = 32; o > 0; o >>= 1) v = fmaxf(v, __shfl_xor(v, o, 64));
    return v;
}

template <typename T> struct Frag;
template <> struct Frag<bf16_t> { bf16x8 v; };
template <> struct Frag<float> { float v[8]; };

__device__ __forceinline__ void mma16(f32x4& acc, const Frag<bf16_t>& a, const Frag<bf16_t>& b) {
    acc = __builtin_amdgcn_mfma_f32_16x16x32_bf16(a.v, b.v, acc, 0, 0, 0);
}
__device__ __forceinline__ void mma16(f32x4& acc, const Frag<float>& a, const Frag<float>& b) {
#pragma unroll
    for (int j = 0; j < 8; ++j) acc = __builtin_amdgcn_mfma_f32_16x16x4f32(a.v[j], b.v[j], acc, 0, 0, 0);
}

typedef __attribute__((address_space(3))) s16x4 lds_s16x4;

__device__ __forceinline__ void frag_load_row(Frag<bf16_t>& f, const unsigned char* p) {
    f.v = *reinterpret_cast<const bf16x8*>(p);
}
__device__ __forceinline__ void frag_load_row(Frag<float>& f, const unsigned char* p) {
    float4 a = *reinterpret_cast<const float4*>(p);
    float4 b = *reinterpret_cast<const float4*>(p + 16);
    f.v[0] = a.x; f.v[1] = a.y; f.v[2] = a.z; f.v[3] = a.w;
    f.v[4] = b.x; f.v[5] = b.y; f.v[6] = b.z; f.v[7] = b.w;
}

__device__ __forceinline__ s16x4 lds_tr16(const unsigned char* p) {
    return __builtin_amdgcn_ds_read_tr16_b64_v4i16((lds_s16x4*)(p));
}
```

### polus_amd/csrc/runtime.hip

```cpp
#include "common.h"
#include <stdarg.h>

static thread_local char g_err[512] = "";

void polus_set_error(const char* fmt, ...) {
    va_list ap;
    va_start(ap, fmt);
    vsnprintf(g_err, sizeof(g_err), fmt, ap);
    va_end(ap);
}

extern "C" const char* polus_last_error(void) { return g_err; }

static PolusCfg g_cfg;
static bool g_cfg_ready = false;
static int env_int(const char* name, int dflt) {
    const char* e = getenv(name);
    return (e && *e) ? atoi(e) : dflt;
}
static void read_cfg() {
    g_cfg.gemm_pp = env_int("POLUS_GEMM_PP", 0);
    g_cfg.gemm_v1 = getenv("POLUS_GEMM_V1") != nullptr;
    g_cfg.dw_ungrouped = getenv("POLUS_DW_UNGROUPED") != nullptr;
    g_cfg.gemm_order = env_int("POLUS_GEMM_ORDER", 4);
    g_cfg.reserve_cus = env_int("POLUS_GEMM_RESERVE_CUS", 0);
    g_cfg.gemm_persist = env_int("POLUS_GEMM_PERSIST", 1);
    g_cfg.dw_fused_reduce = env_int("POLUS_DW_FUSED_REDUCE", 1);
    g_cfg.attn_fused = env_int("POLUS_ATTN_FUSED", 1);
    g_cfg.attn_bwd_kres = env_int("POLUS_ATTN_BWD_KRES", 1);
    g_cfg.attn_debug = env_int("POLUS_ATTN_DEBUG", 0);
    g_cfg.ln_halfwave = env_int("POLUS_LN_HALFWAVE", 1);
    g_cfg.gemm_auto_split = env_int("POLUS_GEMM_AUTO_SPLIT", 1);
    g_cfg.gemm_ring128 = env_int("POLUS_GEMM_RING128", 0);
    g_cfg.ln_bwd_blocks = env_int("POLUS_LN_BWD_BLOCKS", 512);
    g_cfg.ln_fin_single = env_int("POLUS_LN_FIN_SINGLE", 512);
    g_cfg.dw_streamk = env_int("POLUS_DW_STREAMK", 0);
    g_cfg.dw_sk_delta = env_int("POLUS_DW_SK_DELTA", 2);
    g_cfg.dw_sk_cus = env_int("POLUS_DW_SK_CUS", 0);
    g_cfg_ready = true;
}
const PolusCfg& polus_cfg() {
    if (!g_cfg_ready) read_cfg();
    return g_cfg;
}
extern "C" int polus_reload_env(void) { read_cfg(); return POLUS_OK; }

int polus_num_cus() {
    static int n = 0;
    if (!n) {
        int dev = 0; hipDeviceProp_t prop;
        if (hipGetDevice(&dev) == hipSuccess && hipGetDeviceProperties(&prop, dev) == hipSuccess) n = prop.multiProcessorCount;
        if (n <= 0) n = 256;
    }
    return n;
}
static int g_reserve_on = 1;
extern "C" int polus_set_reserve_active(int on) { g_reserve_on = on != 0; return POLUS_OK; }
int polus_reserved_cus() { return g_reserve_on ? polus_cfg().reserve_cus : 0; }

static const PolusDyn* g_dyn = nullptr;
const PolusDyn* polus_dyn() { return g_dyn; }
extern "C" int polus_set_dynamic_params(const void* dev_block16) {
    POLUS_REQUIRE(dev_block16 == nullptr || polus_aligned16(dev_block16), "polus_set_dynamic_params: the block must be 16-byte aligned");
    g_dyn = static_cast<const PolusDyn*>(dev_block16);
    return POLUS_OK;
}
extern "C" int polus_abi_version(void) { return POLUS_ABI_VERSION; }

extern "C" int polus_device_info(int* n_cu, int* lds_bytes_per_cu, char* arch, int arch_len) {
    int dev = 0;
    POLUS_HIP(hipGetDevice(&dev));
    hipDeviceProp_t prop;
    POLUS_HIP(hipGetDeviceProperties(&prop, dev));
    if (n_cu) *n_cu = prop.multiProcessorCount;
    if (lds_bytes_per_cu) *lds_bytes_per_cu = (int)prop.maxSharedMemoryPerMultiProcessor;
    if (arch && arch_len > 0) {
        strncpy(arch, prop.gcnArchName, arch_len - 1);
        arch[arch_len - 1] = 0;
    }
    return POLUS_OK;
}

namespace {

template <typename S, typename D>
__global__ void cast_kernel(const S* __restrict__ src, D* __restrict__ dst, int64_t n) {
    int64_t i4 = ((int64_t)blockIdx.x * blockDim.x + threadIdx.x) * 4;
    const int64_t stride = (int64_t)gridDim.x * blockDim.x * 4;
    for (; i4 < n; i4 += stride) {
        if (i4 + 4 <= n) {
            float v[4];
            load4<S>(src + i4, v);
            store4<D>(dst + i4, v);
        } else {
            for (int64_t j = i4; j < n; ++j) dst[j] = from_f<D>(to_f<S>(src[j]));
        }
    }
}

__global__ void scale_kernel(float* __restrict__ x, float a, int64_t n) {
    int64_t i4 = ((int64_t)blockIdx.x * blockDim.x + threadIdx.x) * 4;
    const int64_t stride = (int64_t)gridDim.x * blockDim.x * 4;
    for (; i4 < n; i4 += stride) {
        if (i4 + 4 <= n) {
            float4 v = *reinterpret_cast<float4*>(x + i4);
            v.x *= a; v.y *= a; v.z *= a; v.w *= a;
            *reinterpret_cast<float4*>(x + i4) = v;
        } else {
            for (int64_t j = i4; j < n; ++j) x[j] *= a;
        }
    }
}

template <typename T>
__global__ void act_bwd_kernel(const T* __restrict__ dy, const T* __restrict__ u, T* __restrict__ du, int64_t n, int act) {
    int64_t i4 = ((int64_t)blockIdx.x * blockDim.x + threadIdx.x) * 4;
    const int64_t stride = (int64_t)gridDim.x * blockDim.x * 4;
    for (; i4 < n; i4 += stride) {
        if (i4 + 4 <= n) {
            float a[4], b[4];
            load4<T>(dy + i4, a);
            load4<T>(u + i4, b);
            apply_act_grad_n<4>(act, a, b);
            store4<T>(du + i4, a);
        } else {
            for (int64_t j = i4; j < n; ++j) { float a1[1] = {to_f<T>(dy[j])}, b1[1] = {to_f<T>(u[j])}; apply_act_grad_n<1>(act, a1, b1); du[j] = from_f<T>(a1[0]); }
        }
    }
}

__global__ __launch_bounds__(256) void transpose16_kernel(const unsigned short* __restrict__ src,
                                                         unsigned short* __restrict__ dst, int R, int C) {
    __shared__ unsigned short tile[64][66];
    const int r0 = blockIdx.y * 64, c0 = blockIdx.x * 64;
    const int tx = threadIdx.x & 63, ty = threadIdx.x >> 6;
    for (int k = ty; k < 64; k += 4) {
        int r = r0 + k, c = c0 + tx;
        tile[k][tx] = (r < R && c < C) ? src[(long)r * C + c] : (unsigned short)0;
    }
    __syncthreads();
    for (int k = ty; k < 64; k += 4) {
        int c = c0 + k, r = r0 + tx;
        if (c < C && r < R) dst[(long)c * R + r] = tile[tx][k];
    }
}

__global__ __launch_bounds__(256) void transpose16_batched_kernel(const unsigned short* __restrict__ src,
                                                                 unsigned short* __restrict__ dst,
                                                                 const long* __restrict__ segs, int nseg) {
    __shared__ unsigned short tile[64][66];
    const int b = blockIdx.x;
    int s = 0;
    while (s + 1 < nseg && segs[4 * (s + 1) + 3] <= b) ++s;
    const long off = segs[4 * s];
    const int R = (int)segs[4 * s + 1], C = (int)segs[4 * s + 2];
    const int t = b - (int)segs[4 * s + 3], tc = (C + 63) / 64;
    const int r0 = (t / tc) * 64, c0 = (t % tc) * 64;
    const unsigned short* sp = src + off;
    unsigned short* dp = dst + off;
    if (((R | C) & 3) == 0) {
        const int q = threadIdx.x & 15, rr = threadIdx.x >> 4;
#pragma unroll
        for (int k = 0; k < 4; ++k) {
            const int r = r0 + rr + 16 * k, c = c0 + 4 * q;
            ushort4 v = make_ushort4(0, 0, 0, 0);
            if (r < R && c < C) v = *reinterpret_cast<const ushort4*>(sp + (long)r * C + c);
            tile[rr + 16 * k][4 * q] = v.x; tile[rr + 16 * k][4 * q + 1] = v.y;
            tile[rr + 16 * k][4 * q + 2] = v.z; tile[rr + 16 * k][4 * q + 3] = v.w;
        }
        __syncthreads();
#pragma unroll
        for (int k = 0; k < 4; ++k) {
            const int c = c0 + rr + 16 * k, r = r0 + 4 * q;
            if (c < C && r < R) {
                ushort4 v = make_ushort4(tile[4 * q][rr + 16 * k], tile[4 * q + 1][rr + 16 * k],
                                         tile[4 * q + 2][rr + 16 * k], tile[4 * q + 3][rr + 16 * k]);
                *reinterpret_cast<ushort4*>(dp + (long)c * R + r) = v;
            }
        }
        return;
    }
    const int tx = threadIdx.x & 63, ty = threadIdx.x >> 6;
    for (int k = ty; k < 64; k += 4) {
        int r = r0 + k, c = c0 + tx;
        tile[k][tx] = (r < R && c < C) ? sp[(long)r * C + c] : (unsigned short)0;
    }
    __syncthreads();
    for (int k = ty; k < 64; k += 4) {
        int c = c0 + k, r = r0 + tx;
        if (c < C && r < R) dp[(long)c * R + r] = tile[tx][k];
    }
}

template <typename T>
__global__ void dropout_kernel(const T* __restrict__ x, T* __restrict__ y, int64_t n, unsigned seed, unsigned thresh, float inv,
                               const PolusDyn* dyn) {
    seed = polus_eff_seed(seed, dyn);
    int64_t i = (int64_t)blockIdx.x * blockDim.x + threadIdx.x;
    const int64_t stride = (int64_t)gridDim.x * blockDim.x;
    for (; i < n; i += stride) y[i] = polus_keep(seed, (unsigned)i, thresh) ? from_f<T>(to_f<T>(x[i]) * inv) : from_f<T>(0.f);
}

__global__ void dropout_mask_kernel(unsigned seed, unsigned thresh, unsigned idx0, int64_t n, uint8_t* __restrict__ mask,
                                    const PolusDyn* dyn) {
    seed = polus_eff_seed(seed, dyn);
    int64_t i = (int64_t)blockIdx.x * blockDim.x + threadIdx.x;
    const int64_t stride = (int64_t)gridDim.x * blockDim.x;
    for (; i < n; i += stride) mask[i] = polus_keep(seed, idx0 + (unsigned)i, thresh) ? 1 : 0;
}

inline int stream_grid(int64_t n) {
    int64_t b = (n / 4 + 255) / 256;
    if (b < 1) b = 1;
    if (b > 2048) b = 2048;
    return (int)b;
}

}

extern "C" int polus_cast(int src_dtype, const void* src, int dst_dtype, void* dst, int64_t n, void* stream) {
    POLUS_REQUIRE(src && dst && n >= 0, "polus_cast: bad arguments");
    if (n == 0) return POLUS_OK;
    POLUS_REQUIRE(((uintptr_t)src % (4 * polus_dtype_size(src_dtype))) == 0 &&
                  ((uintptr_t)dst % (4 * polus_dtype_size(dst_dtype))) == 0,
                  "polus_cast: pointers must be 4-element aligned");
    hipStream_t st = static_cast<hipStream_t>(stream);
    dim3 grid(stream_grid(n)), block(256);
    if (src_dtype == POLUS_F32 && dst_dtype == POLUS_BF16)
        hipLaunchKernelGGL((cast_kernel<float, bf16_t>), grid, block, 0, st, (const float*)src, (bf16_t*)dst, n);
    else if (src_dtype == POLUS_BF16 && dst_dtype == POLUS_F32)
        hipLaunchKernelGGL((cast_kernel<bf16_t, float>), grid, block, 0, st, (const bf16_t*)src, (float*)dst, n);
    else if (src_dtype == POLUS_F32 && dst_dtype == POLUS_F32)
        hipLaunchKernelGGL((cast_kernel<float, float>), grid, block, 0, st, (const float*)src, (float*)dst, n);
    else if (src_dtype == POLUS_BF16 && dst_dtype == POLUS_BF16)
        hipLaunchKernelGGL((cast_kernel<bf16_t, bf16_t>), grid, block, 0, st, (const bf16_t*)src, (bf16_t*)dst, n);
    else POLUS_FAIL("polus_cast: bad dtypes %d -> %d", src_dtype, dst_dtype);
    POLUS_CHECK_LAUNCH("polus_cast");
    return POLUS_OK;
}

extern "C" int polus_scale(float* x, float a, int64_t n, void* stream) {
    POLUS_REQUIRE(x && n >= 0, "polus_scale: bad arguments");
    if (n == 0) return POLUS_OK;
    POLUS_REQUIRE(((uintptr_t)x % 16) == 0, "polus_scale: pointer must be 16-byte aligned");
    hipLaunchKernelGGL(scale_kernel, dim3(stream_grid(n)), dim3(256), 0, static_cast<hipStream_t>(stream), x, a, n);
    POLUS_CHECK_LAUNCH("polus_scale");
    return POLUS_OK;
}

extern "C" int polus_act_bwd(int dtype, const void* dy, const void* u, void* du, int64_t n, int act, void* stream) {
    POLUS_REQUIRE(dy && u && du && n >= 0, "polus_act_bwd: bad arguments");
    if (n == 0) return POLUS_OK;
    size_t es = polus_dtype_size(dtype);
    POLUS_REQUIRE(((uintptr_t)dy % (4 * es)) == 0 && ((uintptr_t)u % (4 * es)) == 0 && ((uintptr_t)du % (4 * es)) == 0,
                  "polus_act_bwd: pointers must be 4-element aligned");
    hipStream_t st = static_cast<hipStream_t>(stream);
    if (dtype == POLUS_BF16)
        hipLaunchKernelGGL(act_bwd_kernel<bf16_t>, dim3(stream_grid(n)), dim3(256), 0, st, (const bf16_t*)dy, (const bf16_t*)u, (bf16_t*)du, n, act);
    else if (dtype == POLUS_F32)
        hipLaunchKernelGGL(act_bwd_kernel<float>, dim3(stream_grid(n)), dim3(256), 0, st, (const float*)dy, (const float*)u, (float*)du, n, act);
    else POLUS_FAIL("polus_act_bwd: bad dtype");
    POLUS_CHECK_LAUNCH("polus_act_bwd");
    return POLUS_OK;
}

extern "C" int polus_transpose_bf16_batched(const void* src_base, void* dst_base, const void* segs_dev, int nseg,
                                            int total_tiles, void* stream) {
    POLUS_REQUIRE(src_base && dst_base && segs_dev && nseg > 0 && total_tiles > 0, "polus_transpose_bf16_batched: bad arguments");
    hipLaunchKernelGGL(transpose16_batched_kernel, dim3(total_tiles), dim3(256), 0, static_cast<hipStream_t>(stream),
                       (const unsigned short*)src_base, (unsigned short*)dst_base, (const long*)segs_dev, nseg);
    POLUS_CHECK_LAUNCH("polus_transpose_bf16_batched");
    return POLUS_OK;
}

extern "C" int polus_transpose_bf16(const void* src, void* dst, int rows, int cols, void* stream) {
    POLUS_REQUIRE(src && dst && rows > 0 && cols > 0, "polus_transpose_bf16: bad arguments");
    dim3 grid((cols + 63) / 64, (rows + 63) / 64);
    hipLaunchKernelGGL(transpose16_kernel, grid, dim3(256), 0, static_cast<hipStream_t>(stream),
                       (const unsigned short*)src, (unsigned short*)dst, rows, cols);
    POLUS_CHECK_LAUNCH("polus_transpose_bf16");
    return POLUS_OK;
}

extern "C" int polus_dropout_mask(uint32_t seed, float drop_p, uint32_t idx0, int64_t n, uint8_t* mask, void* stream) {
    POLUS_REQUIRE(mask && n >= 0 && drop_p >= 0.0f && drop_p < 1.0f, "polus_dropout_mask: bad arguments");
    if (n == 0) return POLUS_OK;
    int64_t b = (n + 255) / 256;
    if (b > 4096) b = 4096;
    hipLaunchKernelGGL(dropout_mask_kernel, dim3((int)b), dim3(256), 0, static_cast<hipStream_t>(stream),
                       seed, polus_drop_thresh(drop_p), idx0, n, mask, polus_dyn());
    POLUS_CHECK_LAUNCH("polus_dropout_mask");
    return POLUS_OK;
}

extern "C" int polus_dropout(int dtype, const void* x, void* y, int64_t n, float drop_p, uint32_t seed, void* stream) {
    POLUS_REQUIRE(x && y && n >= 0 && n < (1LL << 32) && drop_p >= 0.0f && drop_p < 1.0f, "polus_dropout: bad arguments");
    if (n == 0) return POLUS_OK;
    int64_t b = (n + 255) / 256;
    if (b > 4096) b = 4096;
    hipStream_t st = static_cast<hipStream_t>(stream);
    const unsigned th = drop_p > 0.f ? polus_drop_thresh(drop_p) : 0u;
    const float inv = 1.0f / (1.0f - drop_p);
    if (dtype == POLUS_BF16) hipLaunchKernelGGL(dropout_kernel<bf16_t>, dim3((int)b), dim3(256), 0, st, (const bf16_t*)x, (bf16_t*)y, n, seed, th, inv, polus_dyn());
    else if (dtype == POLUS_F32) hipLaunchKernelGGL(dropout_kernel<float>, dim3((int)b), dim3(256), 0, st, (const float*)x, (float*)y, n, seed, th, inv, polus_dyn());
    else POLUS_FAIL("polus_dropout: bad dtype");
    POLUS_CHECK_LAUNCH("polus_dropout");
    return POLUS_OK;
}
```

Measured before the change: 5311.

## Skip trailing padded key blocks in attention forward and backward kernels

Each block scans the attention mask with a wave ballot to find the last live key, then reduces across waves through shared memory to get a key extent. The forward DMA kernel issues and processes only the key blocks up to that extent. The backward kernels skip the matrix multiplies and softmax work for fully padded key tiles, and write zeros into the gradient rows for keys beyond the extent. The aim is to avoid the matmul, exp and data-transfer cost of trailing padding in variable-length NER batches, at the price of a mask scan, extra LDS, more branching, and explicit zero-filling of the skipped gradient outputs.

```diff
diff --git a/polus_amd/csrc/attention.hip b/polus_amd/csrc/attention.hip
--- a/polus_amd/csrc/attention.hip
+++ b/polus_amd/csrc/attention.hip
@@ -93,7 +93,20 @@
     float drop_inv;
     const PolusDyn* dyn;
     int debug;
+    int skip;
 };
+
+__device__ __forceinline__ int fold_last_live(int last, int key, bool live) {
+    const unsigned long long bal = __ballot(live);
+    return bal ? key - (int)(threadIdx.x & 63) + 63 - __clzll((long long)bal) : last;
+}
+template <int NW>
+__device__ __forceinline__ int key_extent(const int* nbw, int full) {
+    int last = -1;
+#pragma unroll
+    for (int w = 0; w < NW; ++w) last = max(last, nbw[w]);
+    return __builtin_amdgcn_readfirstlane(last < 0 ? full : last + 1);
+}
 
 __device__ __forceinline__ float key_bias(const int32_t* mask, int b, int S, int key) {
     if (key >= S) return -INFINITY;
@@ -227,6 +240,7 @@
 
 constexpr int FWD_RING = 4, FWD_STAGE = 2 * BLK * 128;
 constexpr int FWD_MAX_S = 1024;
+__host__ __device__ constexpr int fwd_kbc_len(int S, int NW) { return (S + 64 * NW - 1) / (64 * NW) * 64 * NW; }
 
 template <int NW>
 __global__ __launch_bounds__(64 * NW, NW == 8 ? 4 : 2) void attn_fwd_dma_kernel(AttnArgs p) {
@@ -236,6 +250,7 @@
     extern __shared__ __attribute__((aligned(16))) unsigned char smem[];
     unsigned char* ring = smem;
     float* kbc = reinterpret_cast<float*>(smem + FWD_RING * FWD_STAGE);
+    int* nbw = reinterpret_cast<int*>(kbc + fwd_kbc_len(p.S, NW));
     const int tid = threadIdx.x, lane = tid & 63, i = lane & 15, g = lane >> 4;
     const int wid = __builtin_amdgcn_readfirstlane(tid >> 6);
     const int q0 = blockIdx.x * QB, h = blockIdx.y, b = blockIdx.z;
@@ -277,15 +292,23 @@
         for (int sub = 0; sub < 2; ++sub)
             qf[sub].v = *reinterpret_cast<const bf16x8*>(ring + 3 * FWD_STAGE + row * 128 + (((sub * 4 + g) ^ (row & 7)) * 16));
     }
+    int last = -1;
     for (int t = tid; t < nblk * BLK; t += NT) {
         float bias = 0.0f;
-        if (p.mask) bias = (1.0f - (float)reinterpret_cast<const int*>(kbc)[t]) * MASK_NEG;
+        if (p.mask) {
+            const int mv = reinterpret_cast<const int*>(kbc)[t];
+            bias = (1.0f - (float)mv) * MASK_NEG;
+            last = fold_last_live(last, t, t < S && mv != 0);
+        }
         kbc[t] = t < S ? bias * LOG2E : -INFINITY;
     }
+    if (lane == 0) nbw[wid] = last;
     wait_lgkm();
     __builtin_amdgcn_s_barrier();
-    if (nblk > 3) issue_block(3);
-    int issued = min(nblk, 4);
+    const int nk = p.skip && p.mask ? key_extent<NW>(nbw, nblk * BLK) : nblk * BLK;
+    const int nlive = (nk + BLK - 1) / BLK;
+    if (nlive > 3) issue_block(3);
+    int issued = min(nblk, 3) + (nlive > 3 ? 1 : 0);
 
     const float scale2 = p.scale * LOG2E;
     float m = -1e30f, l = 0.f;
@@ -297,8 +320,9 @@
     const int vrow = 4 * g + (i >> 2), vx = vrow & 7;
     const int v_base = vrow * 128 + (i & 1) * 8, v_c = (i & 3) >> 1;
 
-    for (int j0 = 0; j0 < nblk; j0 += 2) {
-        const bool two = j0 + 1 < nblk;
+    for (int j0 = 0; j0 < nlive; j0 += 2) {
+        const bool two = j0 + 1 < nlive;
+        auto live = [&](int jj, int k16) { return (j0 + jj) * BLK + k16 * 16 < nk; };
         f32x4 s[2][4];
 #pragma unroll
         for (int jj = 0; jj < 2; ++jj) {
@@ -309,6 +333,7 @@
 #pragma unroll
                 for (int kt = 0; kt < 4; ++kt) {
                     s[jj][kt] = (f32x4){0.f, 0.f, 0.f, 0.f};
+                    if (!live(jj, kt)) continue;
                     Frag<T> a0, a1;
                     a0.v = *reinterpret_cast<const bf16x8*>(Kt + kt * 2048 + k_off0);
                     a1.v = *reinterpret_cast<const bf16x8*>(Kt + kt * 2048 + k_off1);
@@ -326,6 +351,7 @@
             if (jj == 0 || two) {
 #pragma unroll
                 for (int kt = 0; kt < 4; ++kt) {
+                    if (!live(jj, kt)) continue;
                     const f32x4 kb = *reinterpret_cast<const f32x4*>(kbc + (j0 + jj) * BLK + kt * 16 + 4 * g);
 #pragma unroll
                     for (int r = 0; r < 4; ++r) s[jj][kt][r] = fmaf(s[jj][kt][r], scale2, kb[r]);
@@ -341,13 +367,16 @@
 #pragma unroll
         for (int jj = 0; jj < 2; ++jj) {
 #pragma unroll
-            for (int kt = 0; kt < 4; ++kt)
+            for (int kt = 0; kt < 4; ++kt) {
+                if (!live(jj, kt)) continue;
 #pragma unroll
                 for (int r = 0; r < 4; ++r) { s[jj][kt][r] = __builtin_amdgcn_exp2f(s[jj][kt][r] - m_new); rs += s[jj][kt][r]; }
+            }
             if (p.drop_thresh) {
                 const unsigned rowb = (((unsigned)b * p.A + h) * S + (unsigned)q) * S + (j0 + jj) * BLK + 4 * g;
 #pragma unroll
                 for (int kt = 0; kt < 4; ++kt) {
+                    if (!live(jj, kt)) continue;
                     float t4[4] = {s[jj][kt][0], s[jj][kt][1], s[jj][kt][2], s[jj][kt][3]};
                     polus_dropout_run<4>(t4, p.drop_seed, rowb + kt * 16, p.drop_thresh, p.drop_inv, (S & 3) == 0);
                     s[jj][kt] = (f32x4){t4[0], t4[1], t4[2], t4[3]};
@@ -369,6 +398,7 @@
                 for (int ks = 0; ks < 2; ++ks)
 #pragma unroll
                     for (int dt = 0; dt < 4; ++dt) {
+                        if (!live(jj, 2 * ks)) continue;
                         const unsigned char* vp = Vt + ks * 4096 + (((2 * dt + v_c) ^ vx) * 16);
                         const s16x4 lo = lds_tr16(vp), hi = lds_tr16(vp + 16 * 128);
                         typedef short s16x8 __attribute__((ext_vector_type(8)));
@@ -379,16 +409,17 @@
                     }
             }
         }
-        if (j0 + 4 < nblk) {
+        if (j0 + 4 < nlive) {
             wait_lgkm();
             __builtin_amdgcn_s_barrier();
             issue_block(j0 + 4);
             ++issued;
-            if (j0 + 5 < nblk) { issue_block(j0 + 5); ++issued; }
+            if (j0 + 5 < nlive) { issue_block(j0 + 5); ++issued; }
         }
     }
     l = col_sum2(l);
     const float inv_l = 1.0f / l;
+    wait_vm<0>();
     wait_lgkm();
     __builtin_amdgcn_s_barrier();
     unsigned char* ot = ring + wid * 2048;
@@ -788,14 +819,14 @@
 template <int NW> struct Q64Cfg {
     static constexpr int S = 16 * NW;
     static constexpr int OFF_O = S * 128, OFF_K = 2 * S * 128, OFF_V = OFF_K + Q64_KB * 128, OFF_P = OFF_V + Q64_KB * 128,
-                         OFF_D = OFF_P + 4 * S * 32, OFF_B = OFF_D + 4 * S * 32, SMEM = OFF_B + S * 4;
+                         OFF_D = OFF_P + 4 * S * 32, OFF_B = OFF_D + 4 * S * 32, OFF_N = OFF_B + S * 4, SMEM = OFF_N + NW * 4;
 };
 
 template <int NW>
 __global__ __launch_bounds__(64 * NW, 4) void attn_bwd_q64_kernel(AttnArgs p) {
     typedef bf16_t T;
     typedef Q64Cfg<NW> C;
-    constexpr int S = C::S, NT = 64 * NW, NKB = S / Q64_KB;
+    constexpr int S = C::S, NT = 64 * NW;
     constexpr int KVP = 16 / NW;
     constexpr int COMBOS = NW >= 8 ? 1 : 8 / NW;
     constexpr int KTW = NW == 16 ? 2 : 4;
@@ -808,6 +839,7 @@
     unsigned char* Ps = smem + C::OFF_P;
     unsigned char* Ds = smem + C::OFF_D;
     float* kbc = reinterpret_cast<float*>(smem + C::OFF_B);
+    int* nbw = reinterpret_cast<int*>(smem + C::OFF_N);
     const int tid = threadIdx.x, lane = tid & 63, i = lane & 15, g = lane >> 4;
     const int wid = __builtin_amdgcn_readfirstlane(tid >> 6);
     const int h = blockIdx.x, b = blockIdx.y;
@@ -835,6 +867,11 @@
     }
     issue_kv(0);
     if (tid < S) kbc[tid] = key_bias(p.mask, b, S, tid) * LOG2E;
+    {
+        const bool live = tid < S && p.skip && p.mask && p.mask[(long)b * S + tid] != 0;
+        const int last = fold_last_live(-1, tid, live);
+        if (lane == 0) nbw[wid] = last;
+    }
     const long stat = ((long)b * p.A + h) * S + q;
     const float lse2 = p.lse[stat] * LOG2E;
     const float scale2 = p.scale * LOG2E;
@@ -847,6 +884,7 @@
     wait_vm<0>();
     wait_lgkm();
     __builtin_amdgcn_s_barrier();
+    const int nk = key_extent<NW>(nbw, S), nlive = (nk + Q64_KB - 1) / Q64_KB;
     const int qoff0 = q * 128 + ((g ^ (q & 7)) * 16), qoff1 = q * 128 + (((4 + g) ^ (q & 7)) * 16);
     float dl = 0.f;
     {
@@ -869,7 +907,7 @@
     const int st_w = q * 32 + ((g ^ ((q >> 2) & 3)) * 8);
     const int st_r = trow * 32 + (((i & 3) ^ g) * 8);
 
-    for (int kb = 0; kb < NKB; ++kb) {
+    for (int kb = 0; kb < nlive; ++kb) {
         f32x4 s[4];
         Frag<T> qf[2], dof[2];
         ds_read128_asm(qf[0], lds_off(Qi + qoff0));
@@ -879,6 +917,13 @@
         const unsigned rowb = (((unsigned)b * p.A + h) * S + (unsigned)q) * S + kb * Q64_KB + 4 * g;
 #pragma unroll
         for (int kt = 0; kt < 4; ++kt) {
+            if (kb * Q64_KB + kt * 16 >= nk) {
+                float z[4] = {0.f, 0.f, 0.f, 0.f};
+                s[kt] = (f32x4){0.f, 0.f, 0.f, 0.f};
+                store4<T>(reinterpret_cast<T*>(Ps + kt * (S * 32) + st_w), z);
+                store4<T>(reinterpret_cast<T*>(Ds + kt * (S * 32) + st_w), z);
+                continue;
+            }
             Frag<T> ka[2], va[2];
             ds_read128_asm(ka[0], lds_off(Kb + kt * 2048 + rr0));
             ds_read128_asm(ka[1], lds_off(Kb + kt * 2048 + rr1));
@@ -919,13 +964,14 @@
             for (int ks = 0; ks < 2; ++ks) {
                 Frag<T> dsb;
                 frag_from_acc(dsb, s[2 * ks], s[2 * ks + 1]);
+                if (kb * Q64_KB + ks * 32 >= nk) continue;
 #pragma unroll
                 for (int dt = 0; dt < 4; ++dt) mma16(dq[dt], kT[ks][dt], dsb);
             }
         }
         wait_lgkm();
         __builtin_amdgcn_s_barrier();
-        if (kb + 1 < NKB) issue_kv(kb + 1);
+        if (kb + 1 < nlive) issue_kv(kb + 1);
 #pragma unroll
         for (int c = 0; c < COMBOS; ++c) {
             const int combo = NW == 16 ? (wid >> 1) : wid * COMBOS + c;
@@ -936,8 +982,9 @@
             f32x4 acc[KTW];
 #pragma unroll
             for (int k2 = 0; k2 < KTW; ++k2) acc[k2] = (f32x4){0.f, 0.f, 0.f, 0.f};
-#pragma unroll
-            for (int q0 = 0; q0 < S / 32; q0 += QH) {
+            const bool tiles_live = kb * Q64_KB + kt0 * 16 < nk;
+#pragma unroll
+            for (int q0 = 0; q0 < S / 32 && tiles_live; q0 += QH) {
                 Frag<T> af[QH];
 #pragma unroll
                 for (int qs = 0; qs < QH; ++qs)
@@ -959,9 +1006,13 @@
                 store4<T>(dqkv + (long)(kb * Q64_KB + (kt0 + k2) * 16 + i) * ld + (type ? 2 * H : H) + h * D + dt * 16 + 4 * g, v);
             }
         }
-        if (kb + 1 < NKB) wait_vm<COMBOS * KTW>();
+        if (kb + 1 < nlive) wait_vm<COMBOS * KTW>();
         wait_lgkm();
         __builtin_amdgcn_s_barrier();
+    }
+    for (int c = nlive * Q64_KB * 16 + tid; c < S * 16; c += NT) {
+        const int row = c >> 4, which = (c >> 3) & 1, ch = c & 7;
+        *reinterpret_cast<uint4*>(dqkv + (long)row * ld + (which ? 2 * H : H) + h * D + ch * 8) = make_uint4(0, 0, 0, 0);
     }
     store_acc_T<T>(dqkv, ld, q, h * D, dq, 1.0f, g, true);
 }
@@ -986,6 +1037,7 @@
     float* lsec = reinterpret_cast<float*>(smem + KR_OFF_STAT);
     const int S = p.S, H = p.H;
     float* deltac = lsec + S;
+    int* nbw = reinterpret_cast<int*>(deltac + S);
     const int tid = threadIdx.x, lane = tid & 63, i = lane & 15, g = lane >> 4;
     const int wid = __builtin_amdgcn_readfirstlane(tid >> 6);
     const int kb = blockIdx.x, h = blockIdx.y, b = blockIdx.z;
@@ -1045,9 +1097,28 @@
     float kb2[2];
 #pragma unroll
     for (int kt = 0; kt < 2; ++kt) kb2[kt] = key_bias(p.mask, b, S, key0 + wid * 32 + kt * 16 + i) * LOG2E;
+    {
+        int last = -1;
+        if (p.skip && p.mask)
+            for (int t = tid; t < S; t += NT) last = fold_last_live(last, t, p.mask[(long)b * S + t] != 0);
+        if (lane == 0) nbw[wid] = last;
+    }
     wait_vm<0>();
     wait_lgkm();
     __builtin_amdgcn_s_barrier();
+    const int nk = key_extent<8>(nbw, S);
+    if (key0 >= nk) {
+        for (int c = tid; c < KR_KEYS * 16; c += NT) {
+            const int row = key0 + (c >> 4), which = (c >> 3) & 1, ch = c & 7;
+            *reinterpret_cast<uint4*>(dqkv + (long)row * ld + (which ? 2 * H : H) + h * D + ch * 8) = make_uint4(0, 0, 0, 0);
+        }
+        if (dq_slabs)
+            for (int c = tid; c < S * (D / 4); c += NT)
+                *reinterpret_cast<float4*>(dq_slabs + ((long)kb * p.B * S + (long)b * S + c / (D / 4)) * H + h * D + (c % (D / 4)) * 4) =
+                    make_float4(0.f, 0.f, 0.f, 0.f);
+        return;
+    }
+    const bool keys_live = key0 + wid * 32 < nk;
 
     const int my_dt = wid & 3, my_qt = wid >> 2;
     Frag<T> kf[2][2], vf[2][2], ktr[8];
@@ -1087,84 +1158,86 @@
     for (int t = 0; t < nsl; ++t) {
         const unsigned char* sl = ring + (t & 3) * 2 * KR_SLICE;
         const int q0 = t * KR_QS;
-        Frag<T> qr[2][2], dor[2][2];
-#pragma unroll
-        for (int qt = 0; qt < 2; ++qt) {
-            ds_read128_asm(qr[qt][0], lds_off(sl + qt * 2048 + rr_off0));
-            ds_read128_asm(qr[qt][1], lds_off(sl + qt * 2048 + rr_off1));
-            ds_read128_asm(dor[qt][0], lds_off(sl + KR_SLICE + qt * 2048 + rr_off0));
-            ds_read128_asm(dor[qt][1], lds_off(sl + KR_SLICE + qt * 2048 + rr_off1));
-        }
-        lds_fence();
-        f32x4 s[2][2], dp[2][2];
-#pragma unroll
-        for (int qt = 0; qt < 2; ++qt)
+        if (keys_live) {
+            Frag<T> qr[2][2], dor[2][2];
+#pragma unroll
+            for (int qt = 0; qt < 2; ++qt) {
+                ds_read128_asm(qr[qt][0], lds_off(sl + qt * 2048 + rr_off0));
+                ds_read128_asm(qr[qt][1], lds_off(sl + qt * 2048 + rr_off1));
+                ds_read128_asm(dor[qt][0], lds_off(sl + KR_SLICE + qt * 2048 + rr_off0));
+                ds_read128_asm(dor[qt][1], lds_off(sl + KR_SLICE + qt * 2048 + rr_off1));
+            }
+            lds_fence();
+            f32x4 s[2][2], dp[2][2];
+#pragma unroll
+            for (int qt = 0; qt < 2; ++qt)
+#pragma unroll
+                for (int kt = 0; kt < 2; ++kt) {
+                    s[qt][kt] = (f32x4){0.f, 0.f, 0.f, 0.f};
+                    dp[qt][kt] = (f32x4){0.f, 0.f, 0.f, 0.f};
+                    mma16(s[qt][kt], qr[qt][0], kf[kt][0]);
+                    mma16(s[qt][kt], qr[qt][1], kf[kt][1]);
+                    mma16(dp[qt][kt], dor[qt][0], vf[kt][0]);
+                    mma16(dp[qt][kt], dor[qt][1], vf[kt][1]);
+                }
+            Frag<T> qT[4], doT[4];
+#pragma unroll
+            for (int dt = 0; dt < 4; ++dt) {
+                const int off = trow * 128 + (((2 * dt + tc) ^ tx) * 16) + thalf;
+                tr_pair_asm<16 * 128>(qT[dt], lds_off(sl + off));
+                tr_pair_asm<16 * 128>(doT[dt], lds_off(sl + KR_SLICE + off));
+            }
+            Frag<T> pf[2], dsf[2];
+            if (!(p.debug & 2))
+#pragma unroll
+            for (int qt = 0; qt < 2; ++qt) {
+                const f32x4 l2 = *reinterpret_cast<const f32x4*>(lsec + q0 + qt * 16 + 4 * g);
+                const f32x4 de = *reinterpret_cast<const f32x4*>(deltac + q0 + qt * 16 + 4 * g);
+#pragma unroll
+                for (int kt = 0; kt < 2; ++kt) {
+                    unsigned h1 = 0, h2 = 0;
+                    if (p.drop_thresh) {
+                        const unsigned key = key0 + wid * 32 + kt * 16 + i;
+                        const unsigned idx = (hash_row + (unsigned)(q0 + qt * 16 + 4 * g + my_r)) * (unsigned)S + (key & ~3u);
+                        h1 = polus_hash32(p.drop_seed, idx >> 2);
+                        h2 = polus_hash32_second(h1);
+                    }
+                    float pd[4], dsv[4];
+#pragma unroll
+                    for (int r = 0; r < 4; ++r) {
+                        const float pr = __builtin_amdgcn_exp2f(fmaf(s[qt][kt][r], scale2, kb2[kt]) - l2[r]);
+                        float pk = pr, dpe = dp[qt][kt][r];
+                        if (p.drop_thresh) {
+                            const unsigned a1 = r == 0 ? quad_bcast<0>(h1) : r == 1 ? quad_bcast<1>(h1) : r == 2 ? quad_bcast<2>(h1) : quad_bcast<3>(h1);
+                            const unsigned a2 = r == 0 ? quad_bcast<0>(h2) : r == 1 ? quad_bcast<1>(h2) : r == 2 ? quad_bcast<2>(h2) : quad_bcast<3>(h2);
+                            const unsigned hh = (i & 2) ? a2 : a1;
+                            const bool keep = ((i & 1) ? (hh >> 16) : (hh & 0xFFFFu)) >= p.drop_thresh;
+                            pk = keep ? pr * p.drop_inv : 0.f;
+                            dpe = keep ? dpe * p.drop_inv : 0.f;
+                        }
+                        pd[r] = pk;
+                        dsv[r] = pr * (dpe - de[r]);
+                    }
+                    s[qt][kt] = (f32x4){pd[0], pd[1], pd[2], pd[3]};
+                    dp[qt][kt] = (f32x4){dsv[0], dsv[1], dsv[2], dsv[3]};
+                    store4<T>(reinterpret_cast<T*>(dsb + (t & 1) * KR_DS + qt * (KR_KEYS * 32) + ds_w[kt]), dsv);
+                }
+            }
 #pragma unroll
             for (int kt = 0; kt < 2; ++kt) {
-                s[qt][kt] = (f32x4){0.f, 0.f, 0.f, 0.f};
-                dp[qt][kt] = (f32x4){0.f, 0.f, 0.f, 0.f};
-                mma16(s[qt][kt], qr[qt][0], kf[kt][0]);
-                mma16(s[qt][kt], qr[qt][1], kf[kt][1]);
-                mma16(dp[qt][kt], dor[qt][0], vf[kt][0]);
-                mma16(dp[qt][kt], dor[qt][1], vf[kt][1]);
-            }
-        Frag<T> qT[4], doT[4];
-#pragma unroll
-        for (int dt = 0; dt < 4; ++dt) {
-            const int off = trow * 128 + (((2 * dt + tc) ^ tx) * 16) + thalf;
-            tr_pair_asm<16 * 128>(qT[dt], lds_off(sl + off));
-            tr_pair_asm<16 * 128>(doT[dt], lds_off(sl + KR_SLICE + off));
-        }
-        Frag<T> pf[2], dsf[2];
-        if (!(p.debug & 2))
-#pragma unroll
-        for (int qt = 0; qt < 2; ++qt) {
-            const f32x4 l2 = *reinterpret_cast<const f32x4*>(lsec + q0 + qt * 16 + 4 * g);
-            const f32x4 de = *reinterpret_cast<const f32x4*>(deltac + q0 + qt * 16 + 4 * g);
-#pragma unroll
-            for (int kt = 0; kt < 2; ++kt) {
-                unsigned h1 = 0, h2 = 0;
-                if (p.drop_thresh) {
-                    const unsigned key = key0 + wid * 32 + kt * 16 + i;
-                    const unsigned idx = (hash_row + (unsigned)(q0 + qt * 16 + 4 * g + my_r)) * (unsigned)S + (key & ~3u);
-                    h1 = polus_hash32(p.drop_seed, idx >> 2);
-                    h2 = polus_hash32_second(h1);
+                frag_from_acc(pf[kt], s[0][kt], s[1][kt]);
+                frag_from_acc(dsf[kt], dp[0][kt], dp[1][kt]);
+            }
+            lds_fence();
+            if (!(p.debug & 4))
+#pragma unroll
+            for (int dt = 0; dt < 4; ++dt)
+#pragma unroll
+                for (int kt = 0; kt < 2; ++kt) {
+                    mma16(dv[dt][kt], doT[dt], pf[kt]);
+                    mma16(dk[dt][kt], qT[dt], dsf[kt]);
                 }
-                float pd[4], dsv[4];
-#pragma unroll
-                for (int r = 0; r < 4; ++r) {
-                    const float pr = __builtin_amdgcn_exp2f(fmaf(s[qt][kt][r], scale2, kb2[kt]) - l2[r]);
-                    float pk = pr, dpe = dp[qt][kt][r];
-                    if (p.drop_thresh) {
-                        const unsigned a1 = r == 0 ? quad_bcast<0>(h1) : r == 1 ? quad_bcast<1>(h1) : r == 2 ? quad_bcast<2>(h1) : quad_bcast<3>(h1);
-                        const unsigned a2 = r == 0 ? quad_bcast<0>(h2) : r == 1 ? quad_bcast<1>(h2) : r == 2 ? quad_bcast<2>(h2) : quad_bcast<3>(h2);
-                        const unsigned hh = (i & 2) ? a2 : a1;
-                        const bool keep = ((i & 1) ? (hh >> 16) : (hh & 0xFFFFu)) >= p.drop_thresh;
-                        pk = keep ? pr * p.drop_inv : 0.f;
-                        dpe = keep ? dpe * p.drop_inv : 0.f;
-                    }
-                    pd[r] = pk;
-                    dsv[r] = pr * (dpe - de[r]);
-                }
-                s[qt][kt] = (f32x4){pd[0], pd[1], pd[2], pd[3]};
-                dp[qt][kt] = (f32x4){dsv[0], dsv[1], dsv[2], dsv[3]};
-                store4<T>(reinterpret_cast<T*>(dsb + (t & 1) * KR_DS + qt * (KR_KEYS * 32) + ds_w[kt]), dsv);
-            }
-        }
-#pragma unroll
-        for (int kt = 0; kt < 2; ++kt) {
-            frag_from_acc(pf[kt], s[0][kt], s[1][kt]);
-            frag_from_acc(dsf[kt], dp[0][kt], dp[1][kt]);
-        }
-        lds_fence();
-        if (!(p.debug & 4))
-#pragma unroll
-        for (int dt = 0; dt < 4; ++dt)
-#pragma unroll
-            for (int kt = 0; kt < 2; ++kt) {
-                mma16(dv[dt][kt], doT[dt], pf[kt]);
-                mma16(dk[dt][kt], qT[dt], dsf[kt]);
-            }
+        }
         {
             const int younger = (t >= 2 ? 1 : 0) + (t + 2 < nsl ? 1 : 0);
             if (younger >= 2) wait_vm<2>(); else if (younger == 1) wait_vm<1>(); else wait_vm<0>();
@@ -1191,7 +1264,8 @@
             for (int ks = 0; ks < 8; ++ks) tr_pair_asm<16 * 32>(dst[ks], base + ks * 32 * 32);
             lds_fence();
 #pragma unroll
-            for (int ks = 0; ks < 8; ++ks) mma16(dq, ktr[ks], dst[ks]);
+            for (int ks = 0; ks < 8; ++ks)
+                if (key0 + ks * 32 < nk) mma16(dq, ktr[ks], dst[ks]);
         }
         dq_prev = dq;
         if (!dq_slabs) {
@@ -1269,7 +1343,7 @@
 template <int NW>
 int launch_fwd_dma(const AttnArgs& a, hipStream_t st) {
     auto kern = attn_fwd_dma_kernel<NW>;
-    const size_t lds = FWD_RING * FWD_STAGE + (size_t)((a.S + 64 * NW - 1) / (64 * NW)) * 64 * NW * 4;
+    const size_t lds = FWD_RING * FWD_STAGE + (size_t)fwd_kbc_len(a.S, NW) * 4 + NW * 4;
     static bool attr_done = false;
     if (!attr_done) {
         POLUS_HIP(hipFuncSetAttribute(reinterpret_cast<const void*>(kern), hipFuncAttributeMaxDynamicSharedMemorySize,
@@ -1320,6 +1394,7 @@
     a.qkv = qkv; a.mask = mask; a.ctx = ctx; a.lse = lse;
     a.B = B; a.S = S; a.A = n_heads; a.H = n_heads * D; a.scale = 0.125f;
     a.drop_thresh = drop_p > 0.f ? polus_drop_thresh(drop_p) : 0u; a.drop_seed = seed; a.drop_inv = 1.0f / (1.0f - drop_p); a.dyn = polus_dyn();
+    a.skip = polus_cfg().attn_skip_padded;
     hipStream_t st = static_cast<hipStream_t>(stream);
     int rc2;
     if (dtype == POLUS_BF16 && S <= FWD_MAX_S)
@@ -1355,13 +1430,14 @@
     POLUS_REQUIRE(drop_p >= 0.f && drop_p < 1.f, "polus_attention_bwd: bad drop_p");
     a.drop_thresh = drop_p > 0.f ? polus_drop_thresh(drop_p) : 0u; a.drop_seed = seed; a.drop_inv = 1.0f / (1.0f - drop_p); a.dyn = polus_dyn();
     a.debug = polus_cfg().attn_debug;
+    a.skip = polus_cfg().attn_skip_padded;
     hipStream_t st = static_cast<hipStream_t>(stream);
     dim3 grid((S + BLK - 1) / BLK, n_heads, B);
     const int kres = polus_cfg().attn_bwd_kres;
     if (dtype == POLUS_BF16 && polus_cfg().attn_fused && kres && S % KR_KEYS == 0 && S <= 2048 && (S > KR_KEYS || kres >= 2)) {
         const int nkb = S / KR_KEYS;
         float* slabs = nkb > 1 ? static_cast<float*>(workspace) + (size_t)B * S * n_heads : nullptr;
-        const size_t lds = KR_OFF_STAT + 2 * (size_t)S * sizeof(float);
+        const size_t lds = KR_OFF_STAT + 2 * (size_t)S * sizeof(float) + 8 * sizeof(int);
         static bool attr_done = false;
         if (!attr_done) {
             POLUS_HIP(hipFuncSetAttribute(reinterpret_cast<const void*>(attn_bwd_kres_kernel), hipFuncAttributeMaxDynamicSharedMemorySize, 160 * 1024));
diff --git a/polus_amd/csrc/common.h b/polus_amd/csrc/common.h
--- a/polus_amd/csrc/common.h
+++ b/polus_amd/csrc/common.h
@@ -42,6 +42,7 @@
     int dw_streamk;
     int dw_sk_cus;
     int dw_sk_delta;
+    int attn_skip_padded;
     int attn_fused;
 };
 const PolusCfg& polus_cfg();
diff --git a/polus_amd/csrc/runtime.hip b/polus_amd/csrc/runtime.hip
--- a/polus_amd/csrc/runtime.hip
+++ b/polus_amd/csrc/runtime.hip
@@ -29,6 +29,7 @@
     g_cfg.attn_fused = env_int("POLUS_ATTN_FUSED", 1);
     g_cfg.attn_bwd_kres = env_int("POLUS_ATTN_BWD_KRES", 1);
     g_cfg.attn_debug = env_int("POLUS_ATTN_DEBUG", 0);
+    g_cfg.attn_skip_padded = env_int("POLUS_ATTN_SKIP_PADDED", 1);
     g_cfg.ln_halfwave = env_int("POLUS_LN_HALFWAVE", 1);
     g_cfg.gemm_auto_split = env_int("POLUS_GEMM_AUTO_SPLIT", 1);
     g_cfg.gemm_ring128 = env_int("POLUS_GEMM_RING128", 0);
```

Result: no change. 5341 (median of 6 runs) (+0.6%).
